# andrewhou1/BlindShadowRemoval

Hardware: AMD Instinct MI355X
Metric: images/sec at 256x256 batch inference (GSC generator forward) (higher is better)
Workload: dtype f32; 1 GPU; BASELINE configs[1]: batch=32 synthetic 256x256x3 per GPU, full GSC generator fp32 (seeded random-init weights in the ckpt-94 variable layout); global_batch=32, height=256, width=256, parallelism=dp1, forwards_in_flight=1, collective=none

## Files before the change

blindshadowremoval_amd/_lib.py:

```python
from __future__ import annotations

import ctypes
import os
from typing import Optional

from . import build as _build
from .build import LIB_PATH

ABI_VERSION = 8
NUM_CLASSES = 7
CLASS_NAMES = ("conv3x3", "convT3x3", "conv1x1", "attention", "conv7", "glue", "convT3x3_ni2")

_lib: Optional[ctypes.CDLL] = None

EXPORTS = ("bsr_create", "bsr_forward", "bsr_forward_tsm", "bsr_workspace_bytes", "bsr_reserve", "bsr_probe", "bsr_set_timing",
           "bsr_get_timing", "bsr_timing_launches", "bsr_timing_entry", "bsr_handle_workspace_bytes", "bsr_debug_attention", "bsr_debug_attention_dtype", "bsr_debug_attention_qw", "bsr_debug_split_qkv", "bsr_clock_trace", "bsr_debug_attention_split", "bsr_destroy", "bsr_last_error", "bsr_abi_version", "bsr_check_range", "bsr_prep_rows", "bsr_prep_groups", "bsr_png_unfilter", "bsr_forward_packed", "bsr_source_sha", "bsr_peek_range", "bsr_png_file_bytes", "bsr_png_scratch_bytes", "bsr_png_encode", "bsr_png_encode_figs", "bsr_ucb_post_scratch_bytes", "bsr_ucb_post",
           "bsr_forward_rgb", "bsr_debug_attention_rgb", "bsr_ucb_post_rgb_scratch_bytes", "bsr_ucb_post_rgb",
           "bsr_sfw_score_scratch_bytes", "bsr_sfw_score", "bsr_ucb_post_tsm_scratch_bytes", "bsr_ucb_post_tsm", "bsr_debug_wino_conv", "bsr_debug_wino_filter", "bsr_debug_keys_compose",
           "bsr_png_unfilter_tall", "bsr_crop_faces")


def load() -> ctypes.CDLL:
    global _lib
    if _lib is not None:
        return _lib
    if not os.path.isfile(LIB_PATH):
        raise RuntimeError("libbsr_hip.so is not built (%s missing): run `python -c 'import __graft_entry__ as g; g.build()'` "
                           "— the HIP path has no fallback" % LIB_PATH)
    try:
        import torch
    except ImportError:
        pass
    lib = ctypes.CDLL(LIB_PATH)
    try:
        lib.bsr_source_sha.restype = ctypes.c_char_p
        built = (lib.bsr_source_sha() or b"").decode()
    except AttributeError:
        built = "<none: built before the hash was embedded>"
    want = _build.source_sha16()
    if built != want:
        raise RuntimeError("libbsr_hip.so is STALE: it was compiled from kernel sources %s, the tree holds %s — rebuild "
                           "(`python -c 'import __graft_entry__ as g; g.build()'`); there is no fallback" % (built, want))
    c_f, c_i, c_v, c_sz = ctypes.POINTER(ctypes.c_float), ctypes.c_int, ctypes.c_void_p, ctypes.c_size_t
    lib.bsr_abi_version.restype = c_i
    lib.bsr_last_error.restype = ctypes.c_char_p
    lib.bsr_create.argtypes = [ctypes.POINTER(c_v), c_i, c_v, c_sz, c_i]
    lib.bsr_create.restype = c_i
    lib.bsr_forward.argtypes = [c_v, c_v, c_v, c_i, c_i, c_i, c_v, c_v, c_v, c_v, c_v]
    lib.bsr_forward.restype = c_i
    lib.bsr_forward_packed.argtypes = [c_v, c_v, c_v, c_i, c_i, c_i, c_v, c_v, c_v, c_v]
    lib.bsr_forward_packed.restype = c_i
    lib.bsr_forward_tsm.argtypes = [c_v, c_v, c_v, c_v, c_i, c_i, c_i, c_i, c_i, c_v, c_v, c_v, c_v, c_v]
    lib.bsr_forward_tsm.restype = c_i
    lib.bsr_forward_rgb.argtypes = [c_v, c_v, c_v, c_i, c_i, c_i, c_v, c_v]
    lib.bsr_forward_rgb.restype = c_i
    lib.bsr_debug_attention_rgb.argtypes = [c_v, c_v, c_i, c_i, c_v]
    lib.bsr_debug_attention_rgb.restype = c_i
    lib.bsr_workspace_bytes.argtypes = [c_i, c_i, c_i]
    lib.bsr_workspace_bytes.restype = c_sz
    lib.bsr_reserve.argtypes = [c_v, c_i, c_i, c_i]
    lib.bsr_reserve.restype = c_i
    lib.bsr_probe.argtypes = [c_v, ctypes.c_char_p, c_v, c_sz, ctypes.POINTER(c_i * 4), c_v]
    lib.bsr_probe.restype = c_i
    lib.bsr_set_timing.argtypes = [c_v, c_i]
    lib.bsr_set_timing.restype = c_i
    lib.bsr_get_timing.argtypes = [c_v, ctypes.POINTER(ctypes.c_float * NUM_CLASSES), ctypes.POINTER(c_i * NUM_CLASSES)]
    lib.bsr_get_timing.restype = c_i
    lib.bsr_timing_launches.argtypes = [c_v]
    lib.bsr_timing_launches.restype = c_i
    lib.bsr_timing_entry.argtypes = [c_v, c_i, ctypes.c_char_p, c_sz, ctypes.POINTER(ctypes.c_float), ctypes.POINTER(c_i)]
    lib.bsr_timing_entry.restype = c_i
    lib.bsr_handle_workspace_bytes.argtypes = [c_v, c_i, c_i, c_i]
    lib.bsr_handle_workspace_bytes.restype = c_sz
    lib.bsr_debug_attention.argtypes = [c_v, c_v, c_i, c_i, c_v]
    lib.bsr_debug_attention.restype = c_i
    lib.bsr_debug_attention_dtype.argtypes = [c_v, c_v, c_i, c_i, c_i, c_v]
    lib.bsr_debug_attention_dtype.restype = c_i
    lib.bsr_debug_attention_qw.argtypes = [c_v, c_v, c_i, c_i, c_i, c_v]
    lib.bsr_clock_trace.argtypes = [c_i, c_v, c_i, c_i, c_v, c_v, c_v]
    lib.bsr_clock_trace.restype = c_i
    lib.bsr_debug_split_qkv.argtypes = [c_v, c_v, c_i, c_i, c_v]
    lib.bsr_debug_split_qkv.restype = c_i
    lib.bsr_debug_attention_split.argtypes = [c_v, c_v, c_i, c_i, c_i, c_v]
    lib.bsr_debug_attention_split.restype = c_i
    lib.bsr_debug_attention_qw.restype = c_i
    lib.bsr_prep_rows.argtypes = [c_i, c_v, c_sz, c_sz, c_sz, c_i, c_i, c_v, c_v, c_v]
    lib.bsr_prep_rows.restype = c_i
    try:
        lib.bsr_prep_groups.argtypes = [c_i, c_v, c_sz, c_sz, c_sz, c_i, c_i, c_i, c_v, c_v, c_v]
    except AttributeError:
        raise RuntimeError("libbsr_hip.so has no bsr_prep_groups: rebuild (`python -c 'import __graft_entry__ as g; g.build()'`); "
                           "there is no fallback") from None
    lib.bsr_prep_groups.restype = c_i
    lib.bsr_png_unfilter.argtypes = [c_i, c_v, c_sz, c_sz, c_i, c_v]
    lib.bsr_png_unfilter.restype = c_i
    try:
        lib.bsr_png_unfilter_tall.argtypes = [c_i, c_v, c_sz, c_sz, c_i, c_v]
        lib.bsr_crop_faces.argtypes = [c_i, c_v, c_sz, c_sz, c_i, c_i, c_v]
    except AttributeError:
        raise RuntimeError("libbsr_hip.so has no bsr_png_unfilter_tall / bsr_crop_faces: rebuild (`python -c 'import __graft_entry__ as g; "
                           "g.build()'`); there is no fallback") from None
    lib.bsr_png_unfilter_tall.restype = c_i
    lib.bsr_crop_faces.restype = c_i
    lib.bsr_check_range.argtypes = [c_v, c_v]
    lib.bsr_check_range.restype = c_i
    lib.bsr_png_file_bytes.argtypes = [c_i, c_i]
    lib.bsr_png_file_bytes.restype = c_sz
    lib.bsr_png_scratch_bytes.argtypes = [c_i]
    lib.bsr_png_scratch_bytes.restype = c_sz
    lib.bsr_png_encode.argtypes = [c_i, c_v, c_i, c_i, c_i, c_v, c_sz, c_v, c_v]
    lib.bsr_png_encode.restype = c_i
    lib.bsr_png_encode_figs.argtypes = [c_i, c_i, c_v, c_v, c_v, c_v, c_v, c_v, c_i, c_i, c_i, c_v, c_sz, c_v, c_v]
    lib.bsr_png_encode_figs.restype = c_i
    lib.bsr_ucb_post_scratch_bytes.argtypes = [c_i, c_i]
    lib.bsr_ucb_post_scratch_bytes.restype = c_sz
    lib.bsr_ucb_post.argtypes = [c_i, c_v, c_v, c_v, c_i, c_i, c_v, c_v, c_v, c_v, c_v, c_v]
    lib.bsr_ucb_post.restype = c_i
    lib.bsr_ucb_post_rgb_scratch_bytes.argtypes = [c_i, c_i]
    lib.bsr_ucb_post_rgb_scratch_bytes.restype = c_sz
    lib.bsr_ucb_post_rgb.argtypes = [c_i, c_v, c_v, c_v, c_i, c_i, c_v, c_v, c_v, c_v, c_v, c_v]
    lib.bsr_ucb_post_rgb.restype = c_i
    lib.bsr_sfw_score_scratch_bytes.argtypes = [c_i, c_i]
    lib.bsr_sfw_score_scratch_bytes.restype = c_sz
    lib.bsr_sfw_score.argtypes = [c_i, c_v, c_i, c_i, c_v, c_v, c_v, c_v, c_v, c_v, c_v]
    lib.bsr_sfw_score.restype = c_i
    lib.bsr_ucb_post_tsm_scratch_bytes.argtypes = [c_i, c_i]
    lib.bsr_ucb_post_tsm_scratch_bytes.restype = c_sz
    lib.bsr_ucb_post_tsm.argtypes = [c_i, c_v, c_v, c_v, c_i, c_i, c_v, c_v, c_v, c_v, c_v, c_v, c_v]
    lib.bsr_ucb_post_tsm.restype = c_i
    lib.bsr_debug_wino_conv.argtypes = [c_v, c_v, c_v, c_v, c_i, c_i, c_i, c_i, c_v]
    lib.bsr_debug_wino_conv.restype = c_i
    lib.bsr_debug_wino_filter.argtypes = [c_v, c_v]
    lib.bsr_debug_wino_filter.restype = c_i
    try:
        lib.bsr_debug_keys_compose.argtypes = [c_v, c_v, c_v, c_v]
    except AttributeError:
        raise RuntimeError("libbsr_hip.so has no bsr_debug_keys_compose: rebuild (`python -c 'import __graft_entry__ as g; g.build()'`); "
                           "there is no fallback") from None
    lib.bsr_debug_keys_compose.restype = c_i
    lib.bsr_peek_range.argtypes = [c_v]
    lib.bsr_peek_range.restype = c_i
    lib.bsr_destroy.argtypes = [c_v]
    lib.bsr_destroy.restype = None
    if lib.bsr_abi_version() != ABI_VERSION:
        raise RuntimeError("libbsr_hip.so ABI %d != binding ABI %d: rebuild" % (lib.bsr_abi_version(), ABI_VERSION))
    _lib = lib
    return lib


def source_sha() -> str:
    return (load().bsr_source_sha() or b"").decode()


class RangeError(RuntimeError):
    """BSR_ERR_RANGE: an activation did not fit fp16 in a forward of a 16-bit-mode handle (include/bsr_hip.h, bsr_check_range)."""


ERR_RANGE = 5


def check(rc: int, what: str) -> None:
    if rc != 0:
        msg = load().bsr_last_error()
        raise (RangeError if rc == ERR_RANGE else RuntimeError)("%s failed (code %d): %s" % (what, rc, msg.decode() if msg else "?"))
```

blindshadowremoval_amd/csrc/attention.h:

```cpp
#pragma once
#include <hip/hip_runtime.h>
#include <type_traits>
#include "igemm_conv.h"
#include "gemm_tail.h"

#ifndef BSR_ATT_PRIO
#define BSR_ATT_PRIO 0
#endif

namespace bsr {

constexpr int kAttD = 128;
constexpr int kAttKT = 32;
constexpr int kAttLdK = kAttD + 4;
constexpr float kRescaleThreshold = 8.f;
constexpr int kAttStageFloats = kAttKT * kAttLdK + kAttKT * kAttD;
constexpr int kAttSmemBytes = 4 * kAttStageFloats * 4;
static_assert(kAttSmemBytes <= 160 * 1024, "LDS budget");
static_assert(66 * 64 * 4 <= 4 * kAttStageFloats, "merge scratch fits the staging buffers");

typedef GemmTailArgs AttWArgs;
typedef GemmTailCfg<5, 4> AttWCfg;
constexpr int kAttWSmemBytes = AttWCfg::SMEM_FLOATS * 4;
static_assert(kAttWSmemBytes <= 160 * 1024 && kAttWSmemBytes >= kAttSmemBytes, "LDS budget of the fused tail");
static_assert(4 * 66 * 64 <= kTailAFloats && kTailLdA == kAttLdK, "the merge scratch sits under the attention tile, clear of the weight ring");

template <int QW, bool FUSEW = false>
__global__ __launch_bounds__(QW * 128, QW == 4 ? 2 : 1) void nonlocal_attention_kernel(const float* __restrict__ qkv, float* __restrict__ out, int tokens, AttWArgs wa) {
  static_assert(!FUSEW || QW == 4, "the fused w tail is the 8-wave shape's");
  extern __shared__ __attribute__((aligned(16))) float smem[];
  constexpr int NT = QW * 128;
  constexpr int SV = 2048 / NT;
  const int tid = threadIdx.x, lane = tid & 63;
  const int wave = __builtin_amdgcn_readfirstlane(tid >> 6);
  const int grp = wave / QW, wq = wave % QW;
  const int h = lane >> 5, r = lane & 31;
  const int qblocks = tokens / (QW * 32);
  int img, qb;
  {
    const int nblk = gridDim.x, b = blockIdx.x;
    const int per_round = 8 * qblocks;
    if (nblk % per_round == 0) {
      const int round = b / per_round, within = b % per_round;
      img = round * 8 + (within % 8);
      qb = within / 8;
    } else {
      img = b / qblocks;
      qb = b % qblocks;
    }
  }
  const float* base = qkv + (size_t)img * tokens * (3 * kAttD);
  const int q = qb * (QW * 32) + wq * 32 + r;
#if BSR_ATT_PRIO
  if (grp == (BSR_ATT_PRIO - 1)) __builtin_amdgcn_s_setprio(2); else __builtin_amdgcn_s_setprio(0);
#endif

  f32x4 qf[kAttD / 8];
#pragma unroll
  for (int g = 0; g < kAttD / 8; ++g)
    qf[g] = *reinterpret_cast<const f32x4*>(base + (size_t)q * (3 * kAttD) + g * 8 + 4 * h) * 1.4426950408889634f;

  f32x16 o[4];
#pragma unroll
  for (int dt = 0; dt < 4; ++dt)
#pragma unroll
    for (int i = 0; i < 16; ++i) o[dt][i] = 0.f;
  float m_run = -INFINITY, l_run = 0.f;

  constexpr int V4_PER_TILE = kAttKT * kAttD / 4;
  constexpr int NV = V4_PER_TILE / NT;
  f32x4 kreg[SV], vreg[SV];
  typedef unsigned u32x4_t __attribute__((ext_vector_type(4)));
  const __amdgpu_buffer_rsrc_t kv_rsrc = make_rsrc(base);
  unsigned kv_voff[NV];
#pragma unroll
  for (int i = 0; i < NV; ++i) {
    const int idx = (tid + i * NT) & (V4_PER_TILE - 1);
    kv_voff[i] = (unsigned)(((idx / (kAttD / 4)) * (3 * kAttD) + (idx % (kAttD / 4)) * 4) * 4);
  }
  auto fetch = [&](int pr) {
#pragma unroll
    for (int i = 0; i < SV; ++i) {
      const unsigned soff = (unsigned)((2 * pr + (i / NV)) * kAttKT * (3 * kAttD) * 4);
      kreg[i] = __builtin_bit_cast(f32x4, (u32x4_t)__builtin_amdgcn_raw_buffer_load_b128(kv_rsrc, kv_voff[i % NV] + (unsigned)(kAttD * 4), soff, 0));
      vreg[i] = __builtin_bit_cast(f32x4, (u32x4_t)__builtin_amdgcn_raw_buffer_load_b128(kv_rsrc, kv_voff[i % NV] + (unsigned)(2 * kAttD * 4), soff, 0));
    }
  };
  auto publish = [&](int pbuf) {
#pragma unroll
    for (int i = 0; i < SV; ++i) {
      const int idx = (tid + i * NT) & (V4_PER_TILE - 1), sel = (tid + i * NT) >> 10;
      const int key = idx / (kAttD / 4), c4 = idx % (kAttD / 4);
      float* sk = smem + (2 * pbuf + sel) * kAttStageFloats;
      float* sv = sk + kAttKT * kAttLdK;
      *reinterpret_cast<f32x4*>(sk + key * kAttLdK + c4 * 4) = kreg[i];
      *reinterpret_cast<f32x4*>(sv + key * kAttD + c4 * 4) = vreg[i];
    }
  };

  const int npair = tokens / (2 * kAttKT);
  fetch(0);
  publish(0);
  __syncthreads();

  auto pair_step = [&](int pr, auto pbuf_const) {
    constexpr int pbuf = decltype(pbuf_const)::value;
    if (pr + 1 < npair) fetch(pr + 1);
    const float* sk = smem + (2 * pbuf + grp) * kAttStageFloats;
    const float* sv = sk + kAttKT * kAttLdK;

    f32x16 s;
#pragma unroll
    for (int i = 0; i < 16; ++i) s[i] = 0.f;
#pragma unroll
    for (int g = 0; g < kAttD / 8; ++g) {
      const f32x4 kf = *reinterpret_cast<const f32x4*>(sk + r * kAttLdK + g * 8 + 4 * h);
#pragma unroll
      for (int j = 0; j < 4; ++j) s = __builtin_amdgcn_mfma_f32_32x32x2f32(kf[j], qf[g][j], s, 0, 0, 0);
    }

    float mx = s[0];
#pragma unroll
    for (int i = 1; i < 16; ++i) mx = fmaxf(mx, s[i]);
    mx = fmaxf(mx, __shfl_xor(mx, 32));
    if (__any(mx > m_run + kRescaleThreshold)) {
      const float m_new = fmaxf(m_run, mx);
      const float scale = __builtin_amdgcn_exp2f(m_run - m_new);
      l_run *= scale;
      m_run = m_new;
#pragma unroll
      for (int dt = 0; dt < 4; ++dt)
#pragma unroll
        for (int i = 0; i < 16; ++i) o[dt][i] *= scale;
    }
    f32x2 ps2 = {0.f, 0.f};
    const f32x2 m2 = {m_run, m_run};
#pragma unroll
    for (int i = 0; i < 16; i += 2) {
      const f32x2 d = f32x2{s[i], s[i + 1]} - m2;
      s[i] = __builtin_amdgcn_exp2f(d[0]);
      s[i + 1] = __builtin_amdgcn_exp2f(d[1]);
      ps2 += f32x2{s[i], s[i + 1]};
    }
    l_run += ps2[0] + ps2[1];

#pragma unroll
    for (int i = 0; i < 16; ++i) {
      const int key = (i & 3) + 8 * (i >> 2) + 4 * h;
      const f32x4 vf = *reinterpret_cast<const f32x4*>(sv + key * kAttD + 4 * r);
#pragma unroll
      for (int dt = 0; dt < 4; ++dt) o[dt] = __builtin_amdgcn_mfma_f32_32x32x2f32(vf[dt], s[i], o[dt], 0, 0, 0);
    }

    if (pr + 1 < npair) {
      publish(pbuf ^ 1);
      __syncthreads();
    }
  };
  for (int pr = 0; pr < npair; pr += 2) {
    pair_step(pr, std::integral_constant<int, 0>{});
    pair_step(pr + 1, std::integral_constant<int, 1>{});
  }

  __syncthreads();
  [[maybe_unused]] float* s_ring = smem + kTailAFloats;
  [[maybe_unused]] float* s_bias = s_ring + 3 * kTailSlot;
  [[maybe_unused]] GemmTailState<5, 4> tail;
  if constexpr (FUSEW) gemm_tail_prefetch(tail, wa, s_bias, tid);
  float* sx = smem + (size_t)wq * 66 * 64 + lane;
  if (grp == 1) {
    sx[0] = m_run;
    sx[64] = l_run;
#pragma unroll
    for (int dt = 0; dt < 4; ++dt)
#pragma unroll
      for (int i = 0; i < 16; ++i) sx[(2 + dt * 16 + i) * 64] = o[dt][i];
  }
  __syncthreads();
  if constexpr (!FUSEW) {
    if (grp == 1) return;
  }
  float inv = 0.f;
  if (grp == 0) {
    const float m1 = sx[0], l1 = sx[64];
    const float m = fmaxf(m_run, m1);
    const float s0 = __builtin_amdgcn_exp2f(m_run - m), s1 = __builtin_amdgcn_exp2f(m1 - m);
    l_run = l_run * s0 + l1 * s1;
#pragma unroll
    for (int dt = 0; dt < 4; ++dt)
#pragma unroll
      for (int i = 0; i < 16; ++i) o[dt][i] = o[dt][i] * s0 + sx[(2 + dt * 16 + i) * 64] * s1;
    const float l_tot = l_run + __shfl_xor(l_run, 32);
    inv = 1.f / l_tot;
  }

  if constexpr (!FUSEW) {
    float* orow = out + ((size_t)img * tokens + q) * kAttD;
#pragma unroll
    for (int i = 0; i < 16; ++i) {
      const int row = (i & 3) + 8 * (i >> 2) + 4 * h;
      f32x4 v = {o[0][i] * inv, o[1][i] * inv, o[2][i] * inv, o[3][i] * inv};
      *reinterpret_cast<f32x4*>(orow + 4 * row) = v;
    }
  } else {
    __syncthreads();
    float* s_att = smem;
    if (grp == 0) {
      float* arow = s_att + (wq * 32 + r) * kTailLdA;
#pragma unroll
      for (int i = 0; i < 16; ++i) {
        const int row = (i & 3) + 8 * (i >> 2) + 4 * h;
        f32x4 v = {o[0][i] * inv, o[1][i] * inv, o[2][i] * inv, o[3][i] * inv};
        *reinterpret_cast<f32x4*>(arow + 4 * row) = v;
      }
    }
    const size_t tile_pix = (size_t)img * tokens + (size_t)qb * 128 + (size_t)__builtin_amdgcn_readfirstlane(wq) * 32;
    gemm_tail_run(tail, wa, s_att, s_ring, s_bias, grp, wq, tile_pix, lane);
  }
}

template <int QW>
inline hipError_t launch_nonlocal_attention_qw(const float* qkv, float* out, int batch, int tokens, hipStream_t stream) {
  auto kern = nonlocal_attention_kernel<QW, false>;
  static PerDeviceOnce once;
  const int dev = PerDeviceOnce::current();
  if (dev < 0 || !once.done[dev]) {
    hipError_t e = hipFuncSetAttribute(reinterpret_cast<const void*>(kern), hipFuncAttributeMaxDynamicSharedMemorySize, kAttSmemBytes);
    if (e != hipSuccess) return e;
    if (dev >= 0) once.done[dev] = true;
  }
  hipLaunchKernelGGL(kern, dim3(batch * (tokens / (QW * 32))), dim3(QW * 128), kAttSmemBytes, stream, qkv, out, tokens, AttWArgs{});
  return hipGetLastError();
}

inline int attention_auto_qw(int batch, int tokens) {
  const long long cus = device_cu_count();
  const long long blocks128 = (long long)batch * (tokens / 128);
  long long best = -1;
  int qw = 4;
  for (int cand : {4, 2, 1}) {
    const long long rounds = (blocks128 * (4 / cand) + cus - 1) / cus;
    const long long cost = rounds * (cand == 4 ? 17 : 10);
    if (best < 0 || cost < best) { best = cost; qw = cand; }
  }
  return qw;
}

inline hipError_t launch_nonlocal_attention_w(const float* qkv, int batch, int tokens, const AttWArgs& wa, hipStream_t stream) {
  if (tokens % (4 * kAttKT) != 0 || wa.n_pad * 32 < AttWCfg::BIAS_FLOATS * 32 || wa.n_pad < 12 * 32 || wa.n_store > 288 || wa.res_c > 288 || wa.out2 != nullptr) return hipErrorInvalidValue;
  auto kern = nonlocal_attention_kernel<4, true>;
  static PerDeviceOnce once;
  const int dev = PerDeviceOnce::current();
  if (dev < 0 || !once.done[dev]) {
    hipError_t e = hipFuncSetAttribute(reinterpret_cast<const void*>(kern), hipFuncAttributeMaxDynamicSharedMemorySize, kAttWSmemBytes);
    if (e != hipSuccess) return e;
    if (dev >= 0) once.done[dev] = true;
  }
  hipLaunchKernelGGL(kern, dim3(batch * (tokens / 128)), dim3(512), kAttWSmemBytes, stream, qkv, static_cast<float*>(nullptr), tokens, wa);
  return hipGetLastError();
}

inline hipError_t launch_nonlocal_attention(const float* qkv, float* out, int batch, int tokens, hipStream_t stream, int qw = 0) {
  if (tokens % (4 * kAttKT) != 0) return hipErrorInvalidValue;
  if (qw == 0) qw = attention_auto_qw(batch, tokens);
  if (qw == 4) return launch_nonlocal_attention_qw<4>(qkv, out, batch, tokens, stream);
  if (qw == 2) return launch_nonlocal_attention_qw<2>(qkv, out, batch, tokens, stream);
  if (qw == 1) return launch_nonlocal_attention_qw<1>(qkv, out, batch, tokens, stream);
  return hipErrorInvalidValue;
}

}
```

blindshadowremoval_amd/csrc/bsr_api.hip:

```cpp
#include "../../include/bsr_hip.h"

#include <hip/hip_runtime.h>
#include <stdint.h>
#include <stdio.h>
#include <stdlib.h>
#include <string.h>

#include <initializer_list>
#include <string>
#include <type_traits>
#include <unordered_map>
#include <vector>

#include "attention.h"
#include "attention256.h"
#include "attention_h16.h"
#include "conv3_f16.h"
#include "conv_n16.h"
#include "gemm_nloop.h"
#include "glue_kernels.h"
#include "igemm_conv.h"
#include "igemm_h16.h"
#include "png_kernels.h"
#include "prep_kernels.h"
#include "prep_group_kernels.h"
#include "rgb_head.h"
#include "stem7.h"
#include "ucb_kernels.h"
#include "ucb_rgb_kernels.h"
#include "ucb_tsm_kernels.h"
#include "sfw_kernels.h"
#include "wino_conv2.h"
#include "wild_crop_kernels.h"

namespace {

thread_local std::string g_last_error;

int fail(int code, const std::string& msg) {
  g_last_error = msg;
  return code;
}

#define HIP_TRY(expr)                                                                              \
  do {                                                                                             \
    hipError_t e__ = (expr);                                                                       \
    if (e__ != hipSuccess)                                                                         \
      return fail(BSR_ERR_HIP, std::string(#expr) + ": " + hipGetErrorString(e__));                \
  } while (0)

struct DeviceGuard {
  int prev = -1;
  hipError_t err = hipSuccess;
  explicit DeviceGuard(int device) {
    if (hipGetDevice(&prev) != hipSuccess) prev = -1;
    if (prev != device) err = hipSetDevice(device);
  }
  ~DeviceGuard() {
    if (prev >= 0) (void)hipSetDevice(prev);
  }
};

bool post_size_ok(int B, int S) { return B > 0 && (S == 32 || S == 64 || S == 128 || S == 256); }

template <class Launch>
int run_post(const char* name, std::initializer_list<const void*> required, int B, int S, const void* scratch, int device, Launch launch) {
  for (const void* p : required)
    if (p == nullptr) return fail(BSR_ERR_ARG, std::string(name) + ": null argument");
  if (!post_size_ok(B, S)) return fail(BSR_ERR_ARG, std::string(name) + ": B must be positive and S one of 32, 64, 128, 256 (reference: 256)");
  if (reinterpret_cast<uintptr_t>(scratch) % 256 != 0) return fail(BSR_ERR_ARG, std::string(name) + ": scratch must be 256-byte aligned");
  DeviceGuard guard(device);
  HIP_TRY(guard.err);
  return launch();
}

constexpr uint32_t kBlobMagic = 0x57525342u;
constexpr uint32_t kBlobVersion = 1;
struct BlobHeader {
  uint32_t magic, version, n_entries, reserved;
};
struct BlobEntry {
  char name[40];
  uint64_t offset;
  uint64_t nfloats;
  int32_t dims[4];
};

struct LayerW {
  const float* w = nullptr;
  const float* b = nullptr;
  int nchunk = 0, taps = 0, n_pad = 0, ldp = 0;
};

enum KClass { K_CONV3 = 0, K_CONVT = 1, K_CONV1 = 2, K_ATT = 3, K_CONV7 = 4, K_GLUE = 5, K_CONVT_NI2 = 6 };

struct Variant {
  bool tsm, rgb;
  int c_a, cs_a, uv_a;
  int c_r, cs_r;
  int c_h, cs_h, uv_h;
  int d = 128, nblk = 6;
  int cs_c3 = 128, cs_c2 = 160;
  int cs_y3x = 288;
  int cs_y = 64, cs_qh = 16;
};
constexpr Variant kGSC{false, false, 99, 120, 96, 257, 264, 261, 264, 258};
constexpr Variant kGSC16{false, false, 99, 128, 96, 257, 288, 261, 288, 258};
constexpr Variant kTSM{true, false, 291, 312, 288, 291, 312, 877, 888, 874};
constexpr Variant kTSM16{true, false, 291, 320, 288, 291, 320, 877, 896, 874};
constexpr Variant kRGB{false, true, 99, 128, 96, 513, 544, 0, 0, 0, 256, 3, 192, 256, 544, 128, 32};
constexpr int CS_Y3X = kGSC.cs_y3x;
constexpr int CS_CF = 64;
constexpr int RGB_CS_R = kRGB.cs_r, RGB_CS_A = kRGB.cs_a, RGB_D = kRGB.d, RGB_CS_C3 = kRGB.cs_c3, RGB_CS_C2 = kRGB.cs_c2, RGB_CS_QH = kRGB.cs_qh;

struct Region {
  size_t off, floats;
};
struct Plan {
  size_t x1, c3, c2, xa, t1, t2, y3[6], qkv, att[6], r[6], xh, ybuf, qh, f1, f2, cf, probe, reg32, share, yh, con, total;
  Region zero[8];
  int nzero;
};

Plan make_plan(size_t B, size_t H, size_t W, const Variant& v) {
  Plan p{};
  size_t off = 0;
  auto take = [&](size_t floats, bool keep_zero = false) {
    size_t o = off;
    off += (floats + 63) & ~size_t(63);
    if (keep_zero && floats != 0) p.zero[p.nzero++] = {o, floats};
    return o;
  };
  const size_t px = B * H * W, cells = px / 64;
  const size_t px2 = v.rgb ? 0 : px;
  const size_t px1 = px - px2;
  p.x1 = take(px * 32);
  p.c3 = take(px / 4 * v.cs_c3);
  p.c2 = take(px / 16 * v.cs_c2);
  p.xa = take(cells * v.cs_a, true);
  p.t1 = take(cells * v.d);
  p.t2 = take(cells * v.d);
  for (int i = 0; i < v.nblk; ++i) p.y3[i] = take(cells * v.cs_y3x);
  p.qkv = take(cells * 3 * v.d);
  for (int i = 0; i < v.nblk; ++i) p.att[i] = take(cells * v.d);
  for (int i = 0; i < v.nblk; ++i) p.r[i] = take(cells * (i < 3 ? v.cs_r : v.cs_h), !v.rgb);
  p.xh = take(cells * v.cs_h, true);
  p.ybuf = take(px * v.cs_y);
  p.qh = take(px * v.cs_qh);
  p.f1 = take(px2 / 16 * 128);
  p.f2 = take(px2 / 4 * 96);
  p.cf = take(px2 * CS_CF);
  p.probe = take(px2 / 64 * 2);
  p.reg32 = take(v.tsm ? cells * 4 : 0);
  p.share = take(v.tsm ? cells * 2 * v.c_r : 0);
  p.yh = take(px1 * 3);
  p.con = take(px1 * 3);
  p.total = off;
  return p;
}

}

struct bsr_handle {
  int device = 0;
  float* d_blob = nullptr;
  float* d_wino = nullptr;
  float* d_keys = nullptr;
  std::unordered_map<std::string, LayerW> layers;
  Variant var = kGSC;
  int dtype = BSR_DTYPE_F32;
  float head_bias[2] = {0.f, 0.f};
  const float* tail_w = nullptr;
  const float* clr_gs_w = nullptr;
  float* ws = nullptr;
  size_t ws_floats = 0;
  Plan plan{};
  const float* rgb_tail_w = nullptr;
  const float* rgb_head_b = nullptr;
  int B = 0, H = 0, W = 0;
  bool ran = false;
  bool att_in_lds = false;
  unsigned* range_flag = nullptr;
  bool fuse_heads = true;
  bool conv1_gemm = true;
  bool att_pv1 = false;
  bool conv3_f16 = true;
  bool fuse_attw = true;
  bool wino_conv2 = true;
  bool keys_conv2 = true;
  bool timing = false;
  std::vector<hipEvent_t> ev;
  std::vector<int> ev_class;
  std::vector<std::string> ev_name;
  size_t ev_used = 0;
};

namespace {

const char* const kRangeMsg =
    "an activation exceeded the fp16 range (|x| >= 65520) in a forward of this 16-bit-mode handle: its outputs are not trustworthy "
    "(inf / NaN where the fp32 path stays finite).  Re-run those inputs on a BSR_DTYPE_F32 handle; bsr_check_range() clears the condition";

constexpr size_t kWinoFloats = 8 * 16 * 128 * 16;
void wino_filter_transform(const float* direct, float* out) {
  static const double G[4][3] = {{1.0, 0.0, 0.0}, {0.5, 0.5, 0.5}, {0.5, -0.5, 0.5}, {0.0, 0.0, 1.0}};
  for (int k = 0; k < 128; ++k)
    for (int n = 0; n < 128; ++n) {
      double t[4][3];
      for (int x = 0; x < 4; ++x)
        for (int b = 0; b < 3; ++b) {
          double acc = 0.0;
          for (int a = 0; a < 3; ++a) acc += G[x][a] * (double)direct[((size_t)((k / 32) * 9 + a * 3 + b) * 128 + n) * 36 + k % 32];
          t[x][b] = acc;
        }
      for (int x = 0; x < 4; ++x)
        for (int y = 0; y < 4; ++y) {
          double acc = 0.0;
          for (int b = 0; b < 3; ++b) acc += t[x][b] * G[y][b];
          out[((size_t)((k / 16) * 16 + 4 * x + y) * 128 + n) * 16 + k % 16] = (float)acc;
        }
    }
}

constexpr int kKeysN = 288 + 256, kKeysNPad = kKeysN + 64, kC3qNPad = 768;
constexpr size_t kKeysFloats = (size_t)4 * kKeysNPad * 36 + kKeysNPad;
void keys_compose(const float* c3q_w, const float* c3q_b, float* out_w, float* out_b) {
  auto src = [&](int k, int n) -> const float& { return c3q_w[((size_t)(k / 32) * kC3qNPad + n) * 36 + k % 32]; };
  memset(out_w, 0, (size_t)4 * kKeysNPad * 36 * sizeof(float));
  memset(out_b, 0, kKeysNPad * sizeof(float));
  for (int ch = 0; ch < 4; ++ch) {
    memcpy(out_w + (size_t)ch * kKeysNPad * 36, c3q_w + (size_t)ch * kC3qNPad * 36, (size_t)288 * 36 * sizeof(float));
    memcpy(out_w + ((size_t)ch * kKeysNPad + 416) * 36, c3q_w + ((size_t)ch * kC3qNPad + 544) * 36, (size_t)128 * 36 * sizeof(float));
  }
  memcpy(out_b, c3q_b, 288 * sizeof(float));
  memcpy(out_b + 416, c3q_b + 544, 128 * sizeof(float));
  for (int m = 0; m < 128; ++m) {
    for (int k = 0; k < 128; ++k) {
      double acc = 0.0;
      for (int c = 0; c < 128; ++c) acc += (double)src(k, 288 + c) * (double)src(m, 416 + c);
      out_w[((size_t)(k / 32) * kKeysNPad + 288 + m) * 36 + k % 32] = (float)acc;
    }
    double acc = 0.0;
    for (int c = 0; c < 128; ++c) acc += (double)c3q_b[288 + c] * (double)src(m, 416 + c);
    out_b[288 + m] = (float)acc;
  }
}

int find_layer(bsr_handle* h, const char* name, int nchunk, int taps, int ldp, int n_min, LayerW* out) {
  auto it = h->layers.find(name);
  if (it == h->layers.end()) return fail(BSR_ERR_BLOB, std::string("blob has no layer '") + name + "'");
  const LayerW& l = it->second;
  if (l.w == nullptr || l.b == nullptr || l.nchunk != nchunk || l.taps != taps || l.ldp != ldp || l.n_pad < n_min) {
    char buf[256];
    snprintf(buf, sizeof buf, "layer '%s': blob has {chunks %d, taps %d, n_pad %d, ldp %d}, kernel needs {%d, %d, >=%d, %d}", name,
             l.nchunk, l.taps, l.n_pad, l.ldp, nchunk, taps, n_min, ldp);
    return fail(BSR_ERR_BLOB, buf);
  }
  *out = l;
  return BSR_OK;
}

template <int V>
using int_c = std::integral_constant<int, V>;
template <class F>
void with_dtype(int dtype, F f) {
  if (dtype == BSR_DTYPE_F32) f(int_c<0>{}, std::false_type{});
  else if (dtype == BSR_DTYPE_F16) f(int_c<2>{}, std::true_type{});
  else f(int_c<2>{}, std::false_type{});
}
template <class F>
void with_io(int io, F f) {
  if (io == 3) f(int_c<3>{});
  else if (io == 2) f(int_c<2>{});
  else if (io == 1) f(int_c<1>{});
  else f(int_c<0>{});
}

bsr::WinoArgs wino_args(const float* in, float* out, const float* w, const float* bias, int H, int W, int out_cs = 128) {
  bsr::WinoArgs a{};
  a.in = in; a.out = out; a.w = w; a.bias = bias; a.H = H; a.W = W; a.in_cs = 128; a.out_cs = out_cs; a.act = 1;
  return a;
}

struct Launcher {
  bsr_handle* h;
  hipStream_t s;
  int rc = BSR_OK;

  void begin(int cls, const char* name) {
    if (!h->timing) return;
    if (h->ev_used + 2 > h->ev.size()) {
      for (int i = 0; i < 2; ++i) {
        hipEvent_t e;
        if (hipEventCreate(&e) != hipSuccess) return;
        h->ev.push_back(e);
      }
      h->ev_class.push_back(cls);
      h->ev_name.emplace_back();
    }
    h->ev_class[h->ev_used / 2] = cls;
    h->ev_name[h->ev_used / 2] = name;
    hipEventRecord(h->ev[h->ev_used], s);
  }
  void end() {
    if (!h->timing || h->ev_used + 2 > h->ev.size()) return;
    hipEventRecord(h->ev[h->ev_used + 1], s);
    h->ev_used += 2;
  }
  void check(hipError_t e, const char* what) {
    if (e != hipSuccess && rc == BSR_OK) rc = fail(BSR_ERR_HIP, std::string(what) + ": " + hipGetErrorString(e));
  }

  template <int KH, int KW, int S, bool TR, int NI, int CC, int INB>
  void conv(int cls, const char* name, const float* in, int in_cs, int in_coff, int k_pad, int H, int W, float* out, int out_cs,
            int out_coff, int n_store, int act, int io = 0) {
    if (rc != BSR_OK) return;
    using C = bsr::ConvCfg<KH, KW, S, TR, 4, 32, 4, 1, 1, NI, CC, INB>;
    constexpr bool k33 = (KH == 3 && KW == 3);
    constexpr bool k11 = (KH == 1 && KW == 1);
    constexpr int CCH = CC == 24 ? 32 : CC;
    const bool h16 = h->dtype != BSR_DTYPE_F32;
    const int nsplit = (k33 && h->dtype == BSR_DTYPE_F16) ? 1 : 2;
    LayerW l;
    const int nb = (n_store + C::BN - 1) / C::BN;
    if (h16) {
      if (k_pad % CCH != 0) { rc = fail(BSR_ERR_ARG, std::string("layer '") + name + "': K is not a multiple of the 16-bit kernels' chunk"); return; }
      const int ldpw = nsplit == 2 ? bsr::H16Cfg<KH, KW, S, TR, 4, 32, 4, 1, 1, NI, CCH, INB, 2>::LDPW : (CCH + 8) / 2;
      rc = find_layer(h, name, k_pad / CCH, KH * KW, ldpw, nb * C::BN, &l);
    } else {
      rc = find_layer(h, name, k_pad / CC, KH * KW, CC + 4, nb * C::BN, &l);
    }
    if (rc != BSR_OK) return;
    bsr::ConvArgs a{};
    a.in = in; a.in_cs = in_cs; a.in_coff = in_coff; a.H = H; a.W = W;
    a.out = out; a.out_cs = out_cs; a.out_coff = out_coff;
    a.Ho = TR ? 2 * H : (H + S - 1) / S;
    a.Wo = TR ? 2 * W : (W + S - 1) / S;
    a.w = l.w; a.bias = l.b; a.nchunk = l.nchunk; a.n_pad = l.n_pad; a.n_store = n_store;
    auto pad_before = [](int in, int k, int s) {
      int o = (in + s - 1) / s, tot = (o - 1) * s + k - in;
      return tot > 0 ? tot / 2 : 0;
    };
    a.pad_t = pad_before(H, KH, S);
    a.pad_l = pad_before(W, KW, S);
    a.act = act;
    a.range_flag = h->range_flag;
    const int mh = TR ? H : a.Ho, mw = TR ? W : a.Wo;
    if (mh % 4 != 0 || mw % 32 != 0) {
      rc = fail(BSR_ERR_ARG, std::string("layer '") + name + "': feature map is not a multiple of the 4x32 tile");
      return;
    }
    if constexpr (k33 && S == 1) {
      if (h->dtype == BSR_DTYPE_F16 && h->conv3_f16) {
        char nm3[48];
        snprintf(nm3, sizeof nm3, "%s.w3", name);
        LayerW l3;
        const int nblk = (n_store + 63) / 64;
        rc = find_layer(h, nm3, nblk * (k_pad / 32), 9, 16, 64, &l3);
        if (rc != BSR_OK) return;
        a.w = l3.w; a.bias = l3.b; a.nchunk = k_pad / 32; a.n_pad = nblk * 64;
        begin(cls, name);
        with_io(io, [&](auto io_c) { check(bsr::launch_conv3_f16<TR, io_c.value>(a, h->B, s), name); });
        end();
        return;
      }
    }
    begin(cls, name);
    static_assert(k33 || k11, "igemm layers are 3x3 or 1x1");
    constexpr bool kTrunk = !TR && S == 1 && NI == 2 && (CC == 32 || (k11 && CC == 24));
    bool half_tile = false;
    if constexpr (kTrunk) half_tile = !h16 && mh % 2 == 0 && (long long)(mh / 4) * (mw / 32) * h->B * nb < bsr::device_cu_count();
    if (half_tile) {
      if constexpr (kTrunk) check(bsr::launch_igemm_conv<KH, KW, S, TR, 2, 32, 2, 2, 1, 1, CC, INB>(a, h->B, s), name);
    } else if (!h16)
      check(bsr::launch_igemm_conv<KH, KW, S, TR, 4, 32, 4, 1, 1, NI, CC, INB>(a, h->B, s), name);
    else if (nsplit == 2)
      check(bsr::launch_igemm_h16<KH, KW, S, TR, 4, 32, 4, 1, 1, NI, CCH, INB, 2>(a, h->B, s), name);
    else if constexpr (k33)
      with_io(io, [&](auto io_c) { check(bsr::launch_igemm_h16<KH, KW, S, TR, 4, 32, 4, 1, 1, NI, CCH, INB, 1, io_c.value>(a, h->B, s), name); });
    end();
  }
  bsr::ConvArgs gemm_args(const LayerW& l, const float* in, int in_cs, float* out, int out_cs, int n_store, int act) const {
    bsr::ConvArgs a{};
    a.in = in; a.in_cs = in_cs; a.out = out; a.out_cs = out_cs;
    a.w = l.w; a.bias = l.b; a.nchunk = l.nchunk; a.n_pad = l.n_pad; a.n_store = n_store; a.act = act;
    a.range_flag = h->range_flag;
    return a;
  }
  template <int NI, int NCH, int MINW = 2>
  void gemm(int cls, const char* name, const float* in, int in_cs, size_t pixels, float* out, int out_cs, int n_store, int act,
            const float* res1 = nullptr, int res1_cs = 0, int res1_c = 0,
            float* out2 = nullptr, int out2_cs = 0, int n_split = 0, int n_store1 = 0, const LayerW* image = nullptr, int out2_gap_at = 0,
            int out2_gap = 0) {
    if (rc != BSR_OK) return;
    using C = bsr::GemmNLoopCfg<NI, NCH>;
    LayerW l;
    const int tiles = (n_store + 31) / 32;
    int kNSplit = 2;
    {
      const long long mblocks = (long long)(pixels / C::BM);
      const int want = (int)((2LL * bsr::device_cu_count() + mblocks - 1) / (mblocks > 0 ? mblocks : 1));
      const int most = (tiles + NI - 1) / NI;
      kNSplit = want < 2 ? 2 : (want > most ? most : want);
#ifdef BSR_NL_NSPLIT
      kNSplit = BSR_NL_NSPLIT > most ? most : BSR_NL_NSPLIT;
#endif
    }
    if (image == nullptr) rc = find_layer(h, name, NCH, 1, 36, (tiles + NI - 1) * 32, &l);
    else if (image->nchunk == NCH && image->ldp == 36 && image->n_pad >= (tiles + NI - 1) * 32) l = *image;
    else rc = fail(BSR_ERR_ARG, std::string("layer '") + name + "': the handle's image does not fit the kernel");
    if (rc != BSR_OK) return;
    if (pixels % C::BM != 0) { rc = fail(BSR_ERR_ARG, std::string("layer '") + name + "': pixel count is not a multiple of 128"); return; }
    bsr::ConvArgs a = gemm_args(l, in, in_cs, out, out_cs, n_store, act);
    a.res1 = res1; a.res1_cs = res1_cs; a.res1_c = res1_c;
    a.out2 = out2; a.out2_cs = out2_cs; a.n_split = n_split; a.n_store1 = n_store1; a.out2_gap_at = out2_gap_at; a.out2_gap = out2_gap;
    a.out2_split = (h->dtype != BSR_DTYPE_F32 && out2 != nullptr) ? 1 : 0;
    begin(cls, name);
    if (h->dtype == BSR_DTYPE_F32)
      check(bsr::launch_gemm_nloop<NI, NCH, 0, MINW>(a, pixels, kNSplit, s), name);
    else if constexpr (MINW == 2)
      check(bsr::launch_gemm_nloop<NI, NCH, 2>(a, pixels, kNSplit, s), name);
    else
      rc = fail(BSR_ERR_ARG, std::string("layer '") + name + "': the RGB bottleneck GEMMs are fp32 only");
    end();
  }
  template <int NCH>
  void gemm_all_n(const char* name, const float* in, size_t pixels, float* out) {
    if (rc != BSR_OK) return;
    LayerW l;
    rc = find_layer(h, name, NCH, 1, 36, 128, &l);
    if (rc != BSR_OK) return;
    begin(K_CONV1, name);
    check(bsr::launch_gemm_nloop<4, NCH, 2, 1>(gemm_args(l, in, NCH * 32, out, 128, 128, 1), pixels, 1, s), name);
    end();
  }

  void stem(const float* in, int H, int W, float* out) {
    if (rc != BSR_OK) return;
    LayerW l;
    rc = find_layer(h, "conv1", 1, 7, h->dtype != BSR_DTYPE_F32 ? 36 : 28, 32, &l);
    if (rc != BSR_OK) return;
    bsr::StemArgs a{in, out, l.w, l.b, H, W, 0, 0, 0, h->range_flag};
    begin(K_CONV7, "conv1");
    with_dtype(h->dtype, [&](auto prec, auto half) { check(bsr::launch_stem7<4, prec.value, half.value>(a, h->B, s), "conv1"); });
    end();
  }

  void wino(const char* name, int i, const float* in, int H, int W, float* out, int out_cs = 128) {
    if (rc != BSR_OK) return;
    LayerW l;
    rc = find_layer(h, name, 4, 9, 36, 128, &l);
    if (rc != BSR_OK) return;
    if (H % 4 != 0 || W % 32 != 0) { rc = fail(BSR_ERR_ARG, std::string("layer '") + name + "': feature map is not a multiple of the 4x32 tile"); return; }
    begin(K_CONV3, name);
    check(bsr::launch_wino_conv2(wino_args(in, out, h->d_wino + (size_t)i * kWinoFloats, l.b, H, W, out_cs), h->B, s), name);
    end();
  }

  void conv71(const char* name, const float* in, int in_cs, int k_pad, int H, int W, float* out, int out_cs) {
    if (rc != BSR_OK) return;
    LayerW l;
    rc = find_layer(h, name, k_pad / 32, 7, 36, 32, &l);
    if (rc != BSR_OK) return;
    if (H % 4 != 0 || W % 32 != 0) { rc = fail(BSR_ERR_ARG, std::string("layer '") + name + "': image is not a multiple of the 4x32 tile"); return; }
    bsr::ConvArgs a{};
    a.in = in; a.in_cs = in_cs; a.in_coff = 0; a.H = H; a.W = W;
    a.out = out; a.out_cs = out_cs; a.out_coff = 0; a.Ho = H; a.Wo = W;
    a.w = l.w; a.bias = l.b; a.nchunk = l.nchunk; a.n_pad = l.n_pad; a.n_store = 32;
    a.pad_t = 3; a.pad_l = 0; a.act = 0;
    begin(K_CONV7, name);
    check(bsr::launch_igemm_conv<7, 1, 1, false, 4, 32, 4, 1, 1, 1, 32, 1>(a, h->B, s), name);
    end();
  }

  void heads(const float* y, int H, int W, float* qh, const float* inputs, float* gs, float* mask22, size_t npix) {
    if (rc != BSR_OK) return;
    LayerW l;
    rc = find_layer(h, "heads", 2, 7, 36, 16, &l);
    if (rc != BSR_OK) return;
    if (l.n_pad != 16) { rc = fail(BSR_ERR_BLOB, "layer 'heads' must be packed with n_pad 16"); return; }
    if (H % 8 != 0 || W % 32 != 0) { rc = fail(BSR_ERR_ARG, "layer 'heads': image is not a multiple of its tile"); return; }
    bsr::ConvN16Args a{};
    a.in = y; a.in_cs = 64; a.H = H; a.W = W; a.w = l.w; a.bias = l.b; a.out = qh; a.out_cs = 16; a.act = 0;
    a.pad_t = 3; a.pad_l = 0;
    a.inputs = inputs; a.gs_out = gs; a.mask22 = mask22; a.b_mask = h->head_bias[0]; a.b_con = h->head_bias[1];
    a.range_flag = h->range_flag;
    int resident = 0;
    check(bsr::launch_conv_n16<7, 1, false, false, 2, 0, false, true>(a, h->B, s, &resident), "heads");
    const bool fuse = rc == BSR_OK && h->fuse_heads && bsr::conv_n16_fuse_pays(h->B, H, 8, resident);
    begin(K_CONV7, "heads");
    with_dtype(h->dtype, [&](auto prec, auto half) {
      if (fuse) check(bsr::launch_conv_n16<7, 1, false, false, 2, prec.value, half.value, true>(a, h->B, s), "heads");
      else check(bsr::launch_conv_n16<7, 1, false, false, 2, prec.value, half.value>(a, h->B, s), "heads");
    });
    end();
    if (fuse) return;
    begin(K_GLUE, "heads_post");
    hipLaunchKernelGGL(bsr::heads_post_kernel, dim3((unsigned)((npix + 255) / 256)), dim3(256), 0, s, qh, inputs, h->head_bias[0], h->head_bias[1], gs,
                       mask22, W, npix);
    check(hipGetLastError(), "heads_post");
    end();
  }

  template <int KH, int KW, bool GS, bool TAIL, int RW>
  void conv16(int cls, const char* name, const float* in, int in_cs, int H, int W, float* out, int out_cs, int act, const float* gs,
              const float* inputs, float* con_rgb, float* dif, float* packed = nullptr) {
    if (rc != BSR_OK) return;
    LayerW l;
    rc = find_layer(h, name, 2, KH * KW, 36, 16, &l);
    if (rc != BSR_OK) return;
    if (l.n_pad != 16) { rc = fail(BSR_ERR_BLOB, std::string("layer '") + name + "' must be packed with n_pad 16"); return; }
    bsr::ConvN16Args a{};
    a.in = in; a.in_cs = in_cs; a.H = H; a.W = W; a.w = l.w; a.bias = l.b; a.out = out; a.out_cs = out_cs; a.act = act;
    a.pad_t = (KH - 1) / 2; a.pad_l = (KW - 1) / 2;
    a.gs = gs; a.w_gs = h->clr_gs_w; a.tail_w = h->tail_w; a.inputs = inputs; a.con_rgb = con_rgb; a.dif = dif; a.packed = packed;
    a.range_flag = h->range_flag;
    if (H % (4 * RW) != 0 || W % 32 != 0) { rc = fail(BSR_ERR_ARG, std::string("layer '") + name + "': image is not a multiple of its tile"); return; }
    begin(cls, name);
    with_dtype(h->dtype, [&](auto prec, auto half) { check(bsr::launch_conv_n16<KH, KW, GS, TAIL, RW, prec.value, half.value>(a, h->B, s), name); });
    end();
  }
};

int grow_workspace(bsr_handle* h, size_t floats, bool device_wide, hipStream_t s) {
  if (floats <= h->ws_floats) return BSR_OK;
  if (device_wide) HIP_TRY(hipDeviceSynchronize());
  else HIP_TRY(hipStreamSynchronize(s));
  if (h->ws) HIP_TRY(hipFree(h->ws));
  h->ws = nullptr;
  h->ws_floats = 0;
  HIP_TRY(hipMalloc(reinterpret_cast<void**>(&h->ws), floats * sizeof(float)));
  h->ws_floats = floats;
  h->B = 0;
  h->ran = false;
  if (device_wide) HIP_TRY(hipMemset(h->ws, 0, floats * sizeof(float)));
  else HIP_TRY(hipMemsetAsync(h->ws, 0, floats * sizeof(float), s));
  return BSR_OK;
}

int ensure_workspace(bsr_handle* h, int B, int H, int W, hipStream_t s) {
  const Plan p = make_plan(B, H, W, h->var);
  const bool fresh = p.total > h->ws_floats;
  const int rc = grow_workspace(h, p.total, false, s);
  if (rc != BSR_OK) return rc;
  if (!fresh && (B != h->B || H != h->H || W != h->W)) {
    for (int i = 0; i < p.nzero; ++i) HIP_TRY(hipMemsetAsync(h->ws + p.zero[i].off, 0, p.zero[i].floats * sizeof(float), s));
    h->ran = false;
  }
  h->plan = p;
  h->B = B; h->H = H; h->W = W;
  return BSR_OK;
}

template <typename T>
int read_records(const unsigned char* blob, size_t off, int n, hipStream_t s, std::vector<T>* out) {
  out->resize((size_t)n);
  HIP_TRY(hipMemcpyAsync(out->data(), blob + off, (size_t)n * sizeof(T), hipMemcpyDeviceToHost, s));
  HIP_TRY(hipStreamSynchronize(s));
  return BSR_OK;
}

}

extern "C" {

int bsr_abi_version(void) { return 8; }

#ifndef BSR_SRC_SHA
#define BSR_SRC_SHA "unhashed"
#endif
static const char kSrcShaTag[] = "BSR_SRC_SHA=" BSR_SRC_SHA;
const char* bsr_source_sha(void) { return kSrcShaTag + 12; }

const char* bsr_last_error(void) { return g_last_error.c_str(); }

size_t bsr_workspace_bytes(int B, int H, int W) {
  if (B <= 0 || H <= 0 || W <= 0) return 0;
  return make_plan(B, H, W, kGSC).total * sizeof(float);
}

int bsr_create(bsr_handle** out, int device, const void* packed_weights, size_t nbytes, int dtype) {
  if (out == nullptr || packed_weights == nullptr) return fail(BSR_ERR_ARG, "bsr_create: null argument");
  *out = nullptr;
  if (dtype != BSR_DTYPE_F32 && dtype != BSR_DTYPE_F16 && dtype != BSR_DTYPE_F32X3)
    return fail(BSR_ERR_ARG, "bsr_create: dtype must be BSR_DTYPE_F32, BSR_DTYPE_F16 or BSR_DTYPE_F32X3");
  if (nbytes < sizeof(BlobHeader)) return fail(BSR_ERR_BLOB, "bsr_create: blob shorter than its header");
  const uint8_t* blob = static_cast<const uint8_t*>(packed_weights);
  BlobHeader hd;
  memcpy(&hd, blob, sizeof hd);
  if (hd.magic != kBlobMagic || hd.version != kBlobVersion) return fail(BSR_ERR_BLOB, "bsr_create: bad blob magic/version");
  if ((int)hd.reserved != dtype) return fail(BSR_ERR_BLOB, "bsr_create: the blob was packed for another dtype (pack_generator(weights, dtype) must match bsr_create's dtype)");
  const size_t table_end = sizeof(BlobHeader) + (size_t)hd.n_entries * sizeof(BlobEntry);
  if (table_end > nbytes) return fail(BSR_ERR_BLOB, "bsr_create: blob entry table exceeds blob size");
  DeviceGuard guard(device);
  HIP_TRY(guard.err);
  bsr_handle* h = new bsr_handle();
  h->device = device;
  h->dtype = dtype;
  h->att_pv1 = dtype == BSR_DTYPE_F16;
  const struct { const char* env; bool* on; } switches[] = {{"BSR_FUSE_HEADS", &h->fuse_heads}, {"BSR_FUSE_ATTW", &h->fuse_attw}, {"BSR_CONV3_F16", &h->conv3_f16},
                                                            {"BSR_CONV1_GEMM", &h->conv1_gemm}, {"BSR_WINO_CONV2", &h->wino_conv2},
                                                            {"BSR_KEYS_CONV2", &h->keys_conv2}};
  for (const auto& sw : switches)
    if (const char* e_ = getenv(sw.env)) *sw.on = atoi(e_) != 0;
  hipError_t e = hipMalloc(reinterpret_cast<void**>(&h->d_blob), nbytes);
  if (e == hipSuccess) e = hipMemcpy(h->d_blob, blob, nbytes, hipMemcpyHostToDevice);
  if (e != hipSuccess) {
    if (h->d_blob) hipFree(h->d_blob);
    delete h;
    return fail(BSR_ERR_HIP, std::string("bsr_create: weight upload: ") + hipGetErrorString(e));
  }
  for (uint32_t i = 0; i < hd.n_entries; ++i) {
    BlobEntry en;
    memcpy(&en, blob + sizeof(BlobHeader) + (size_t)i * sizeof(BlobEntry), sizeof en);
    en.name[sizeof(en.name) - 1] = 0;
    if (en.offset % 16 != 0 || en.offset + en.nfloats * 4 > nbytes) {
      bsr_destroy(h);
      return fail(BSR_ERR_BLOB, std::string("bsr_create: entry '") + en.name + "' is out of bounds or misaligned");
    }
    std::string nm(en.name);
    const float* dptr = reinterpret_cast<const float*>(reinterpret_cast<const uint8_t*>(h->d_blob) + en.offset);
    if (nm == "heads.bias") {
      if (en.nfloats != 2) { bsr_destroy(h); return fail(BSR_ERR_BLOB, "bsr_create: heads.bias must hold 2 floats"); }
      memcpy(h->head_bias, blob + en.offset, 8);
    } else if (nm == "clr_conv1.gs") {
      if (en.nfloats != 256) { bsr_destroy(h); return fail(BSR_ERR_BLOB, "bsr_create: clr_conv1.gs must hold 16x16 floats"); }
      h->clr_gs_w = dptr;
    } else if (nm == "rgb.tail") {
      if (en.nfloats != 7 * 7 * 3 * 3 + 3) { bsr_destroy(h); return fail(BSR_ERR_BLOB, "bsr_create: rgb.tail must hold 7x7x3x3 + 3 floats"); }
      h->rgb_tail_w = dptr;
    } else if (nm == "rgb.head_bias") {
      if (en.nfloats != 3) { bsr_destroy(h); return fail(BSR_ERR_BLOB, "bsr_create: rgb.head_bias must hold 3 floats"); }
      h->rgb_head_b = dptr;
    } else if (nm == "tail.w") {
      if (en.nfloats != 16 * 16 + 16 + 48 + 3) { bsr_destroy(h); return fail(BSR_ERR_BLOB, "bsr_create: tail.w has the wrong size"); }
      h->tail_w = dptr;
    } else if (nm.size() > 2 && nm.compare(nm.size() - 2, 2, ".w") == 0) {
      LayerW& l = h->layers[nm.substr(0, nm.size() - 2)];
      l.w = dptr;
      l.nchunk = en.dims[0]; l.taps = en.dims[1]; l.n_pad = en.dims[2]; l.ldp = en.dims[3];
      if ((uint64_t)l.nchunk * l.taps * l.n_pad * l.ldp != en.nfloats) {
        bsr_destroy(h);
        return fail(BSR_ERR_BLOB, std::string("bsr_create: entry '") + en.name + "' dims do not match its size");
      }
    } else if (nm.size() > 2 && nm.compare(nm.size() - 2, 2, ".b") == 0) {
      h->layers[nm.substr(0, nm.size() - 2)].b = dptr;
    }
  }
  if (h->layers.count("rgb_head") != 0) {
    if (dtype != BSR_DTYPE_F32) {
      bsr_destroy(h);
      return fail(BSR_ERR_ARG, "bsr_create: these are RGB-baseline weights (model_RGB.py), which run in BSR_DTYPE_F32 only: BSR_DTYPE_F32X3 and BSR_DTYPE_F16 are not provided for them");
    }
    if (h->rgb_tail_w == nullptr || h->rgb_head_b == nullptr) { bsr_destroy(h); return fail(BSR_ERR_BLOB, "bsr_create: RGB blob lacks 'rgb.tail' / 'rgb.head_bias'"); }
    h->var = kRGB;
    *out = h;
    return BSR_OK;
  }
  if (h->tail_w == nullptr || h->clr_gs_w == nullptr) { bsr_destroy(h); return fail(BSR_ERR_BLOB, "bsr_create: blob lacks 'tail.w' / 'clr_conv1.gs'"); }
  if (dtype != BSR_DTYPE_F32) {
    e = hipHostMalloc(reinterpret_cast<void**>(&h->range_flag), 64, hipHostMallocMapped);
    if (e != hipSuccess) { h->range_flag = nullptr; bsr_destroy(h); return fail(BSR_ERR_HIP, std::string("bsr_create: range flag: ") + hipGetErrorString(e)); }
    *h->range_flag = 0u;
  }
  {
    auto it = h->layers.find("res0.conv1");
    if (it == h->layers.end()) { bsr_destroy(h); return fail(BSR_ERR_BLOB, "bsr_create: blob has no 'res0.conv1'"); }
    const int nch = it->second.nchunk;
    if (dtype == BSR_DTYPE_F32) h->var = nch == 13 ? kTSM : kGSC;
    else h->var = nch == 10 ? kTSM16 : kGSC16;
  }
  if (dtype == BSR_DTYPE_F32) {
    std::vector<float> u(6 * kWinoFloats);
    for (int i = 0; i < 6; ++i) {
      char nm[32];
      snprintf(nm, sizeof nm, "res%d.conv2", i);
      LayerW l;
      if (find_layer(h, nm, 4, 9, 36, 128, &l) != BSR_OK || l.n_pad != 128) { bsr_destroy(h); return fail(BSR_ERR_BLOB, std::string("bsr_create: layer '") + nm + "' is not a [4][9][128][36] image"); }
      wino_filter_transform(reinterpret_cast<const float*>(blob + (reinterpret_cast<const uint8_t*>(l.w) - reinterpret_cast<const uint8_t*>(h->d_blob))), u.data() + i * kWinoFloats);
    }
    e = hipMalloc(reinterpret_cast<void**>(&h->d_wino), u.size() * sizeof(float));
    if (e == hipSuccess) e = hipMemcpy(h->d_wino, u.data(), u.size() * sizeof(float), hipMemcpyHostToDevice);
    if (e != hipSuccess) { bsr_destroy(h); return fail(BSR_ERR_HIP, std::string("bsr_create: Winograd weights: ") + hipGetErrorString(e)); }
    std::vector<float> q(6 * kKeysFloats);
    auto host = [&](const float* dev) { return reinterpret_cast<const float*>(blob + (reinterpret_cast<const uint8_t*>(dev) - reinterpret_cast<const uint8_t*>(h->d_blob))); };
    for (int i = 0; i < 6; ++i) {
      char nm[32];
      snprintf(nm, sizeof nm, "res%d.c3q", i);
      LayerW l;
      if (find_layer(h, nm, 4, 1, 36, kC3qNPad, &l) != BSR_OK || l.n_pad != kC3qNPad) { bsr_destroy(h); return fail(BSR_ERR_BLOB, std::string("bsr_create: layer '") + nm + "' is not a [4][1][768][36] image"); }
      keys_compose(host(l.w), host(l.b), q.data() + i * kKeysFloats, q.data() + i * kKeysFloats + (size_t)4 * kKeysNPad * 36);
    }
    e = hipMalloc(reinterpret_cast<void**>(&h->d_keys), q.size() * sizeof(float));
    if (e == hipSuccess) e = hipMemcpy(h->d_keys, q.data(), q.size() * sizeof(float), hipMemcpyHostToDevice);
    if (e != hipSuccess) { bsr_destroy(h); return fail(BSR_ERR_HIP, std::string("bsr_create: composed c3q weights: ") + hipGetErrorString(e)); }
  }
  *out = h;
  return BSR_OK;
}

void bsr_destroy(bsr_handle* h) {
  if (h == nullptr) return;
  DeviceGuard guard(h->device);
  for (hipEvent_t e : h->ev) hipEventDestroy(e);
  if (h->ws) hipFree(h->ws);
  if (h->d_blob) hipFree(h->d_blob);
  if (h->d_wino) hipFree(h->d_wino);
  if (h->d_keys) hipFree(h->d_keys);
  if (h->range_flag) hipHostFree(h->range_flag);
  delete h;
}

int bsr_reserve(bsr_handle* h, int B, int H, int W) {
  if (h == nullptr || B <= 0 || H <= 0 || W <= 0) return fail(BSR_ERR_ARG, "bsr_reserve: bad argument");
  DeviceGuard guard(h->device);
  HIP_TRY(guard.err);
  return grow_workspace(h, make_plan(B, H, W, h->var).total, true, nullptr);
}

int bsr_check_range(bsr_handle* h, void* stream) {
  if (h == nullptr) return fail(BSR_ERR_ARG, "bsr_check_range: null handle");
  if (h->range_flag == nullptr) return BSR_OK;
  DeviceGuard guard(h->device);
  HIP_TRY(guard.err);
  HIP_TRY(hipStreamSynchronize(static_cast<hipStream_t>(stream)));
  if (__atomic_exchange_n(h->range_flag, 0u, __ATOMIC_SEQ_CST) == 0u) return BSR_OK;
  return fail(BSR_ERR_RANGE, kRangeMsg);
}

int bsr_peek_range(bsr_handle* h) {
  if (h == nullptr) return fail(BSR_ERR_ARG, "bsr_peek_range: null handle");
  if (h->range_flag == nullptr) return BSR_OK;
  if (__atomic_load_n(h->range_flag, __ATOMIC_SEQ_CST) == 0u) return BSR_OK;
  return fail(BSR_ERR_RANGE, kRangeMsg);
}

int bsr_set_timing(bsr_handle* h, int enable) {
  if (h == nullptr) return fail(BSR_ERR_ARG, "bsr_set_timing: null handle");
  h->timing = enable != 0;
  h->ev_used = 0;
  return BSR_OK;
}

int bsr_get_timing(bsr_handle* h, float ms[BSR_NUM_CLASSES], int launches[BSR_NUM_CLASSES]) {
  if (h == nullptr || ms == nullptr || launches == nullptr) return fail(BSR_ERR_ARG, "bsr_get_timing: null argument");
  for (int i = 0; i < BSR_NUM_CLASSES; ++i) { ms[i] = 0.f; launches[i] = 0; }
  for (size_t i = 0; i + 1 < h->ev_used; i += 2) {
    HIP_TRY(hipEventSynchronize(h->ev[i + 1]));
    float t = 0.f;
    HIP_TRY(hipEventElapsedTime(&t, h->ev[i], h->ev[i + 1]));
    const int c = h->ev_class[i / 2];
    ms[c] += t;
    launches[c] += 1;
  }
  return BSR_OK;
}

int bsr_timing_launches(bsr_handle* h) { return h == nullptr ? 0 : (int)(h->ev_used / 2); }

int bsr_timing_entry(bsr_handle* h, int i, char* name, size_t name_cap, float* ms, int* cls) {
  if (h == nullptr || name == nullptr || ms == nullptr || cls == nullptr || name_cap == 0) return fail(BSR_ERR_ARG, "bsr_timing_entry: null argument");
  if (i < 0 || (size_t)(2 * i + 1) >= h->ev_used) return fail(BSR_ERR_ARG, "bsr_timing_entry: index out of range");
  HIP_TRY(hipEventSynchronize(h->ev[2 * i + 1]));
  HIP_TRY(hipEventElapsedTime(ms, h->ev[2 * i], h->ev[2 * i + 1]));
  *cls = h->ev_class[i];
  snprintf(name, name_cap, "%s", h->ev_name[i].c_str());
  return BSR_OK;
}

size_t bsr_handle_workspace_bytes(const bsr_handle* h, int B, int H, int W) {
  if (h == nullptr || B <= 0 || H <= 0 || W <= 0) return 0;
  return make_plan(B, H, W, h->var).total * sizeof(float);
}

static int check_image_size(int H, int W, const char* hw_text, const char* token_text) {
  if (H <= 0 || W <= 0 || H % 32 != 0 || W % 256 != 0) return fail(BSR_ERR_ARG, hw_text);
  if (((H / 8) * (W / 8)) % 128 != 0) return fail(BSR_ERR_ARG, token_text);
  return BSR_OK;
}
#define BSR_CHECK_IMAGE_SIZE(entry, H, W)                                                                                          \
  check_image_size(H, W, entry ": H must be a multiple of 32 and W a multiple of 256 (reference: 256x256)",                         \
                   entry ": (H/8)*(W/8) must be a multiple of 128")

static int forward_impl(bsr_handle* h, const float* inputs, const float* uv, const float* reg, int frame, int share, int B, int H, int W,
                        float* gs, float* con_rgb, float* mask22, float* dif, void* stream, float* packed = nullptr) {
  if (h == nullptr || inputs == nullptr || uv == nullptr || gs == nullptr || mask22 == nullptr || (packed == nullptr && (con_rgb == nullptr || dif == nullptr)))
    return fail(BSR_ERR_ARG, "bsr_forward: null argument");
  if (B <= 0) return fail(BSR_ERR_ARG, "bsr_forward: B must be positive");
  const Variant& V = h->var;
  if (V.rgb)
    return fail(BSR_ERR_ARG, reg != nullptr ? "bsr_forward_tsm: this handle holds RGB-baseline weights: call bsr_forward_rgb"
                                            : "bsr_forward: this handle holds RGB-baseline weights: call bsr_forward_rgb");
  if (V.tsm != (reg != nullptr))
    return fail(BSR_ERR_ARG, V.tsm ? "bsr_forward: this handle holds TSM weights: call bsr_forward_tsm" : "bsr_forward_tsm: this handle holds GSC weights: call bsr_forward");
  if (V.tsm && (frame <= 0 || B % frame != 0 || H != W))
    return fail(BSR_ERR_ARG, "bsr_forward_tsm: B must be a multiple of frame and the image square (warp.py assumes a square map)");
  int rc = BSR_CHECK_IMAGE_SIZE("bsr_forward", H, W);
  if (rc != BSR_OK) return rc;
  hipStream_t s = static_cast<hipStream_t>(stream);
  if (h->range_flag != nullptr && *reinterpret_cast<volatile unsigned*>(h->range_flag) != 0u)
    return fail(BSR_ERR_RANGE, kRangeMsg);
  DeviceGuard guard(h->device);
  HIP_TRY(guard.err);
  rc = ensure_workspace(h, B, H, W, s);
  if (rc != BSR_OK) return rc;
  h->ev_used = 0;
  const Plan& p = h->plan;
  float* ws = h->ws;
  const size_t npix = (size_t)B * H * W, ncell = npix / 64;
  const int H2 = H / 2, W2 = W / 2, H4 = H / 4, W4 = W / 4, H8 = H / 8, W8 = W / 8;
  Launcher L{h, s};
  auto glue_begin = [&](const char* what) { L.begin(K_GLUE, what); };
  auto glue_end = [&](const char* what) { L.check(hipGetLastError(), what); L.end(); };

  L.stem(inputs, H, W, ws + p.x1);
  const bool p16 = h->dtype == BSR_DTYPE_F16;
  const int io_both = p16 ? 3 : 0, io_in = p16 ? 1 : 0, io_out = p16 ? 2 : 0;
  L.conv<3, 3, 2, false, 2, 16, 1>(K_CONV3, "down1", ws + p.x1, 32, 0, 32, H, W, ws + p.c3, 128, 64, 64, 1, io_both);
  L.conv<3, 3, 2, false, 2, 16, 1>(K_CONV3, "down2", ws + p.c3, 128, 64, 64, H2, W2, ws + p.c2, 160, 96, 64, 1, io_both);
  L.conv<3, 3, 2, false, 3, 16, 1>(K_CONV3, "down3", ws + p.c2, 160, 96, 64, H4, W4, ws + p.xa, V.cs_a, 0, 96, 1, io_in);
  glue_begin("uv_resize8");
  hipLaunchKernelGGL(bsr::uv_resize8_kernel, dim3((unsigned)((ncell * 3 + 255) / 256)), dim3(256), 0, s, uv, H, W, ws + p.xa, V.cs_a, V.uv_a,
                     ws + p.xh, V.cs_h, V.uv_h, ncell);
  glue_end("uv_resize8");

  auto share_layer = [&](const float* x, int x_cs, int C, float* out, int out_cs, int out_coff) {
    glue_begin("share_layer");
    if (share) hipLaunchKernelGGL(bsr::share_reduce_kernel, dim3((unsigned)(ncell / frame)), dim3(128), 0, s, x, x_cs, C, ws + p.reg32, H8, frame, ws + p.share);
    hipLaunchKernelGGL(bsr::share_unwarp_kernel, dim3((unsigned)ncell), dim3(128), 0, s, ws + p.share, x, x_cs, C, ws + p.reg32, H8, frame, share, out, out_cs, out_coff);
    glue_end("share_layer");
  };
  if (V.tsm) {
    glue_begin("reg_resize8");
    hipLaunchKernelGGL(bsr::reg_resize8_kernel, dim3((unsigned)((ncell * 4 + 255) / 256)), dim3(256), 0, s, reg, H, W, ws + p.reg32, ncell);
    glue_end("reg_resize8");
    share_layer(ws + p.xa, V.cs_a, 96, ws + p.xa, V.cs_a, 96);
  }

  auto conv1_gemm = [&](const char* nm, const float* x, int x_cs) -> bool {
    if (V.tsm || !h->conv1_gemm || L.rc != BSR_OK) return false;
    if (h->dtype == BSR_DTYPE_F32) return false;
    if (ncell % 128 != 0 || (long long)(ncell / 128) * 2 < bsr::device_cu_count()) return false;
    if (x_cs != 128 && x_cs != 288) return false;
    if (x_cs == 128) L.gemm_all_n<4>(nm, x, ncell, ws + p.t1);
    else L.gemm_all_n<9>(nm, x, ncell, ws + p.t1);
    return true;
  };

  auto res_block = [&](int i, const float* x, int x_cs, int x_c) {
    float* r_out = ws + p.r[i];
    const int o_cs = i < 3 ? V.cs_r : V.cs_h;
    char nm[32];
    float* y3 = ws + p.y3[i];
    snprintf(nm, sizeof nm, "res%d.conv1", i);
    if (!conv1_gemm(nm, x, x_cs)) L.conv<1, 1, 1, false, 2, 24, 3>(K_CONV1, nm, x, x_cs, 0, x_cs, H8, W8, ws + p.t1, 128, 0, 128, 1);
    const bool keys = h->dtype == BSR_DTYPE_F32 && h->keys_conv2;
    float* t2_row = keys ? ws + p.qkv : ws + p.t2;
    const int t2_cs = keys ? 384 : 128, t2_coff = keys ? 128 : 0;
    float* t2 = t2_row + t2_coff;
    snprintf(nm, sizeof nm, "res%d.conv2", i);
    if (h->dtype == BSR_DTYPE_F32 && h->wino_conv2) L.wino(nm, i, ws + p.t1, H8, W8, t2, t2_cs);
    else L.conv<3, 3, 1, false, 2, 32, 1>(K_CONV3, nm, ws + p.t1, 128, 0, 128, H8, W8, t2_row, t2_cs, t2_coff, 128, 1);
    snprintf(nm, sizeof nm, "res%d.c3q", i);
    if (keys) {
      const float* img = h->d_keys + (size_t)i * kKeysFloats;
      const LayerW lk{img, img + (size_t)4 * kKeysNPad * 36, 4, 1, kKeysNPad, 36};
      L.gemm<3, 4>(K_CONV1, nm, t2, t2_cs, ncell, y3, CS_Y3X, kKeysN, 0, x, x_cs, x_cs < 288 ? x_cs : 288, ws + p.qkv, 384, 288, CS_Y3X, &lk, 128, 128);
    } else {
      L.gemm<3, 4>(K_CONV1, nm, t2, t2_cs, ncell, y3, CS_Y3X, 288 + 384, 0, x, x_cs, x_cs < 288 ? x_cs : 288, ws + p.qkv, 384, 288, CS_Y3X);
    }
    const bool h16 = h->dtype != BSR_DTYPE_F32;
    const bool fuse_w = h->fuse_attw && (h16 || bsr::attention_auto_qw(B, H8 * W8) == 4);
    h->att_in_lds = fuse_w;
    if (fuse_w && L.rc == BSR_OK) {
      LayerW l;
      snprintf(nm, sizeof nm, h16 ? "res%d.w4" : "res%d.w", i);
      L.rc = h16 ? find_layer(h, nm, 9, 1, 128, 32, &l) : find_layer(h, nm, 4, 1, 36, 12 * 32, &l);
      if (L.rc == BSR_OK) {
        bsr::AttWArgs wa{};
        wa.w = l.w; wa.bias = l.b; wa.n_pad = h16 ? 288 : l.n_pad;
        wa.res = y3; wa.res_cs = CS_Y3X; wa.res_c = CS_Y3X;
        wa.out = r_out; wa.out_cs = o_cs; wa.n_store = o_cs < 288 ? o_cs : 288; wa.n_store1 = wa.n_store; wa.act = 1; wa.stagger = 1;
        snprintf(nm, sizeof nm, "res%d.attw", i);
        L.begin(K_ATT, nm);
        if (!h16)
          L.check(bsr::launch_nonlocal_attention_w(ws + p.qkv, B, H8 * W8, wa, s), "attention+w");
        else
          L.check(bsr::launch_nonlocal_attention_h16_w(ws + p.qkv, B, H8 * W8, wa, s, h->att_pv1), "attention_h16+w");
        L.end();
      }
    } else {
      if (L.rc == BSR_OK) {
        snprintf(nm, sizeof nm, "res%d.attention", i);
        L.begin(K_ATT, nm);
        if (!h16)
          L.check(bsr::launch_nonlocal_attention(ws + p.qkv, ws + p.att[i], B, H8 * W8, s), "attention");
        else
          L.check(bsr::launch_nonlocal_attention_h16(ws + p.qkv, ws + p.att[i], B, H8 * W8, s, h->att_pv1), "attention_h16");
        L.end();
      }
      snprintf(nm, sizeof nm, "res%d.w", i);
      L.gemm<3, 4>(K_CONV1, nm, ws + p.att[i], 128, ncell, r_out, o_cs, o_cs < 288 ? o_cs : 288, 1, y3, CS_Y3X, CS_Y3X);
    }
    if (x_c > 288 && L.rc == BSR_OK) {
      glue_begin("lrelu_copy");
      hipLaunchKernelGGL(bsr::lrelu_copy_kernel, dim3((unsigned)((ncell * (x_c - 288) + 255) / 256)), dim3(256), 0, s, x, x_cs, r_out, o_cs, 288, x_c, ncell);
      glue_end("lrelu_copy");
    }
  };
  res_block(0, ws + p.xa, V.cs_a, V.c_a);
  res_block(1, ws + p.r[0], V.cs_r, V.c_r);
  res_block(2, ws + p.r[1], V.cs_r, V.c_r);

  L.conv<3, 3, 1, true, 1, 24, 1>(K_CONVT, "up1", ws + p.r[2], V.cs_r, 0, V.cs_r, H8, W8, ws + p.c2, 160, 0, 96, 1, io_out);
  L.conv<3, 3, 1, true, 2, 32, 1>(K_CONVT_NI2, "up2", ws + p.c2, 160, 0, 160, H4, W4, ws + p.c3, 128, 0, 64, 1, io_both);
  L.conv<3, 3, 1, true, 2, 32, 1>(K_CONVT_NI2, "up3", ws + p.c3, 128, 0, 128, H2, W2, ws + p.ybuf, 64, 0, 64, 1, io_both);
  L.heads(ws + p.ybuf, H, W, ws + p.qh, inputs, gs, mask22, npix);
  glue_begin("bmask_xhole");
  hipLaunchKernelGGL(bsr::bmask_xhole_kernel, dim3((unsigned)ncell), dim3(64), 0, s, gs, inputs, H, W, ws + p.r[2], V.cs_r, V.c_r, ws + p.xh,
                     V.cs_h, ws + p.probe);
  glue_end("bmask_xhole");
  if (V.tsm) share_layer(ws + p.xh, V.cs_h, V.c_r, ws + p.xh, V.cs_h, V.c_r + 1);

  res_block(3, ws + p.xh, V.cs_h, V.c_h);
  res_block(4, ws + p.r[3], V.cs_h, V.c_h);
  res_block(5, ws + p.r[4], V.cs_h, V.c_h);

  L.conv<3, 3, 1, true, 2, 24, 1>(K_CONVT, "clr_up1", ws + p.r[5], V.cs_h, 0, V.cs_h, H8, W8, ws + p.f1, 128, 0, 128, 1, io_out);
  L.conv<3, 3, 1, true, 1, 32, 1>(K_CONVT, "clr_up2", ws + p.f1, 128, 0, 128, H4, W4, ws + p.f2, 96, 0, 96, 1, io_both);
  L.conv<3, 3, 1, true, 2, 32, 1>(K_CONVT_NI2, "clr_up3", ws + p.f2, 96, 0, 96, H2, W2, ws + p.cf, CS_CF, 0, 64, 1, io_both);
  L.conv16<3, 3, true, true, 2>(K_CONV3, "clr_conv1", ws + p.cf, CS_CF, H, W, nullptr, 0, 1, gs, inputs, con_rgb, dif, packed);
  if (L.rc == BSR_OK) h->ran = true;
  return L.rc;
}

int bsr_forward_rgb(bsr_handle* h, const float* inputs, const float* uv, int B, int H, int W, float* con, void* stream) {
  if (h == nullptr || inputs == nullptr || uv == nullptr || con == nullptr) return fail(BSR_ERR_ARG, "bsr_forward_rgb: null argument");
  if (!h->var.rgb)
    return fail(BSR_ERR_ARG, h->var.tsm ? "bsr_forward_rgb: this handle holds TSM weights: call bsr_forward_tsm"
                                        : "bsr_forward_rgb: this handle holds GSC weights: call bsr_forward");
  if (B <= 0) return fail(BSR_ERR_ARG, "bsr_forward_rgb: B must be positive");
  int rc = BSR_CHECK_IMAGE_SIZE("bsr_forward_rgb", H, W);
  if (rc != BSR_OK) return rc;
  hipStream_t s = static_cast<hipStream_t>(stream);
  DeviceGuard guard(h->device);
  HIP_TRY(guard.err);
  rc = ensure_workspace(h, B, H, W, s);
  if (rc != BSR_OK) return rc;
  h->ev_used = 0;
  h->att_in_lds = false;
  const Plan& p = h->plan;
  float* ws = h->ws;
  const size_t npix = (size_t)B * H * W, ncell = npix / 64;
  const int H2 = H / 2, W2 = W / 2, H4 = H / 4, W4 = W / 4, H8 = H / 8, W8 = W / 8;
  Launcher L{h, s};
  auto glue_begin = [&](const char* what) { L.begin(K_GLUE, what); };
  auto glue_end = [&](const char* what) { L.check(hipGetLastError(), what); L.end(); };

  L.stem(inputs, H, W, ws + p.x1);
  L.conv<3, 3, 2, false, 2, 16, 1>(K_CONV3, "down1", ws + p.x1, 32, 0, 32, H, W, ws + p.c3, RGB_CS_C3, 128, 64, 1);
  L.conv<3, 3, 2, false, 2, 16, 1>(K_CONV3, "down2", ws + p.c3, RGB_CS_C3, 128, 64, H2, W2, ws + p.c2, RGB_CS_C2, 192, 64, 1);
  L.conv<3, 3, 2, false, 3, 16, 1>(K_CONV3, "down3", ws + p.c2, RGB_CS_C2, 192, 64, H4, W4, ws + p.xa, RGB_CS_A, 0, 96, 1);
  glue_begin("uv_resize8");
  hipLaunchKernelGGL(bsr::uv_resize8_kernel, dim3((unsigned)((ncell * 3 + 255) / 256)), dim3(256), 0, s, uv, H, W, ws + p.xa, RGB_CS_A, 96,
                     ws + p.xa, RGB_CS_A, 96, ncell);
  glue_end("uv_resize8");

  auto res_block = [&](int i, const float* x, int x_cs) {
    char nm[32];
    float* y3 = ws + p.y3[i];
    snprintf(nm, sizeof nm, "res%d.conv1", i);
    L.conv<1, 1, 1, false, 2, 32, 3>(K_CONV1, nm, x, x_cs, 0, x_cs, H8, W8, ws + p.t1, RGB_D, 0, RGB_D, 1);
    snprintf(nm, sizeof nm, "res%d.conv2", i);
    L.conv<3, 3, 1, false, 2, 32, 1>(K_CONV3, nm, ws + p.t1, RGB_D, 0, RGB_D, H8, W8, ws + p.t2, RGB_D, 0, RGB_D, 1);
    snprintf(nm, sizeof nm, "res%d.c3q", i);
    L.gemm<3, 8, 1>(K_CONV1, nm, ws + p.t2, RGB_D, ncell, y3, RGB_CS_R, RGB_CS_R + 3 * RGB_D, 0, x, x_cs, x_cs, ws + p.qkv, 3 * RGB_D, RGB_CS_R,
                    RGB_CS_R);
    if (L.rc == BSR_OK) {
      snprintf(nm, sizeof nm, "res%d.attention", i);
      L.begin(K_ATT, nm);
      L.check(bsr::launch_nonlocal_attention256(ws + p.qkv, ws + p.att[i], B, H8 * W8, s), "attention256");
      L.end();
    }
    snprintf(nm, sizeof nm, "res%d.w", i);
    L.gemm<3, 8, 1>(K_CONV1, nm, ws + p.att[i], RGB_D, ncell, ws + p.r[i], RGB_CS_R, RGB_CS_R, 1, y3, RGB_CS_R, RGB_CS_R);
  };
  res_block(0, ws + p.xa, RGB_CS_A);
  res_block(1, ws + p.r[0], RGB_CS_R);
  res_block(2, ws + p.r[1], RGB_CS_R);

  L.conv<3, 3, 1, true, 2, 32, 1>(K_CONVT, "up1", ws + p.r[2], RGB_CS_R, 0, RGB_CS_R, H8, W8, ws + p.c2, RGB_CS_C2, 0, 192, 1);
  L.conv<3, 3, 1, true, 2, 32, 1>(K_CONVT_NI2, "up2", ws + p.c2, RGB_CS_C2, 0, RGB_CS_C2, H4, W4, ws + p.c3, RGB_CS_C3, 0, 128, 1);
  L.conv<3, 3, 1, true, 2, 32, 1>(K_CONVT_NI2, "up3", ws + p.c3, RGB_CS_C3, 0, RGB_CS_C3, H2, W2, ws + p.ybuf, 128, 0, 128, 1);
  L.conv71("rgb_head", ws + p.ybuf, 128, 128, H, W, ws + p.qh, RGB_CS_QH);
  if (L.rc == BSR_OK) {
    glue_begin("rgb_hsum");
    hipLaunchKernelGGL(bsr::rgb_hsum_kernel, dim3((unsigned)((npix * 3 + 255) / 256)), dim3(256), 0, s, ws + p.qh, RGB_CS_QH, h->rgb_head_b, W,
                       ws + p.yh, npix);
    glue_end("rgb_hsum");
    L.begin(K_CONV7, "rgb_tail");
    L.check(bsr::launch_rgb_conv7(ws + p.yh, h->rgb_tail_w, B, H, W, con, ws + p.con, s), "rgb_tail");
    L.end();
  }
  if (L.rc == BSR_OK) h->ran = true;
  return L.rc;
}

int bsr_forward(bsr_handle* h, const float* inputs, const float* uv, int B, int H, int W, float* gs, float* con_rgb, float* mask22,
                float* dif, void* stream) {
  return forward_impl(h, inputs, uv, nullptr, 1, 0, B, H, W, gs, con_rgb, mask22, dif, stream);
}

int bsr_forward_packed(bsr_handle* h, const float* inputs, const float* uv, int B, int H, int W, float* gs, float* con_rgb_dif, float* mask22,
                       void* stream) {
  if (con_rgb_dif == nullptr) return fail(BSR_ERR_ARG, "bsr_forward_packed: null con_rgb_dif");
  return forward_impl(h, inputs, uv, nullptr, 1, 0, B, H, W, gs, nullptr, mask22, nullptr, stream, con_rgb_dif);
}

int bsr_forward_tsm(bsr_handle* h, const float* inputs, const float* uv, const float* reg, int B, int H, int W, int frame, int share,
                    float* gs, float* con_rgb, float* mask22, float* dif, void* stream) {
  if (reg == nullptr) return fail(BSR_ERR_ARG, "bsr_forward_tsm: null reg");
  return forward_impl(h, inputs, uv, reg, frame, share != 0, B, H, W, gs, con_rgb, mask22, dif, stream);
}

int bsr_prep_rows(int device, const void* d_blob, size_t blob_bytes, size_t rows_off, size_t grid_off, int B, int S, float* out, float* hull_tmp,
                  void* stream) {
  if (d_blob == nullptr || out == nullptr || hull_tmp == nullptr) return fail(BSR_ERR_ARG, "bsr_prep_rows: null argument");
  if (B <= 0 || S <= 0 || (S * S) % 256 != 0) return fail(BSR_ERR_ARG, "bsr_prep_rows: B must be positive and S*S a multiple of 256");
  if (rows_off % 8 != 0 || grid_off % 8 != 0) return fail(BSR_ERR_ARG, "bsr_prep_rows: table offsets must be 8-byte aligned");
  if (rows_off > blob_bytes || (size_t)B * sizeof(bsr::PrepRow) > blob_bytes - rows_off || grid_off > blob_bytes ||
      (size_t)S * sizeof(double) > blob_bytes - grid_off)
    return fail(BSR_ERR_ARG, "bsr_prep_rows: the row / grid tables do not fit in blob_bytes");
  DeviceGuard guard(device);
  HIP_TRY(guard.err);
  hipStream_t s = static_cast<hipStream_t>(stream);
  const unsigned char* blob = static_cast<const unsigned char*>(d_blob);
  const dim3 grid((unsigned)(S * S / 256), (unsigned)B);
  hipLaunchKernelGGL(bsr::prep_rows_kernel, grid, dim3(256), 0, s, blob, reinterpret_cast<const bsr::PrepRow*>(blob + rows_off),
                     reinterpret_cast<const double*>(blob + grid_off), S, out, hull_tmp);
  HIP_TRY(hipGetLastError());
  hipLaunchKernelGGL(bsr::prep_blur_kernel, grid, dim3(256), 0, s, hull_tmp, S, 16, out);
  HIP_TRY(hipGetLastError());
  return BSR_OK;
}

int bsr_prep_groups(int device, const void* d_blob, size_t blob_bytes, size_t groups_off, size_t grid_off, int B, int S, int planes, float* out,
                    float* hull_tmp, void* stream) {
  if (d_blob == nullptr || out == nullptr || hull_tmp == nullptr) return fail(BSR_ERR_ARG, "bsr_prep_groups: null argument");
  if (B <= 0 || S <= 0 || (S * S) % 256 != 0) return fail(BSR_ERR_ARG, "bsr_prep_groups: B must be positive and S*S a multiple of 256");
  if (planes != 6 && planes != 7) return fail(BSR_ERR_ARG, "bsr_prep_groups: planes must be 6 (img3, gt3) or 7 (img3, cmap3, label1)");
  if (groups_off % 8 != 0 || grid_off % 8 != 0) return fail(BSR_ERR_ARG, "bsr_prep_groups: table offsets must be 8-byte aligned");
  if (groups_off > blob_bytes || (size_t)B * sizeof(bsr::PrepGroup) > blob_bytes - groups_off || grid_off > blob_bytes ||
      (size_t)S * sizeof(double) > blob_bytes - grid_off)
    return fail(BSR_ERR_ARG, "bsr_prep_groups: the group / grid tables do not fit in blob_bytes");
  DeviceGuard guard(device);
  HIP_TRY(guard.err);
  hipStream_t s = static_cast<hipStream_t>(stream);
  const unsigned char* blob = static_cast<const unsigned char*>(d_blob);
  const bsr::PrepGroup* groups = reinterpret_cast<const bsr::PrepGroup*>(blob + groups_off);
  const double* lin = reinterpret_cast<const double*>(blob + grid_off);
  const dim3 grid((unsigned)(S * S / 256), (unsigned)B);
  if (planes == 6)
    hipLaunchKernelGGL(bsr::prep_groups_kernel<6>, grid, dim3(256), 0, s, blob, groups, lin, S, out, hull_tmp);
  else
    hipLaunchKernelGGL(bsr::prep_groups_kernel<7>, grid, dim3(256), 0, s, blob, groups, lin, S, out, hull_tmp);
  HIP_TRY(hipGetLastError());
  hipLaunchKernelGGL(bsr::prep_blur_kernel, dim3((unsigned)(S * S / 256), 2u * (unsigned)B), dim3(256), 0, s, hull_tmp, S, planes + 10, out);
  HIP_TRY(hipGetLastError());
  return BSR_OK;
}

int bsr_png_unfilter(int device, void* d_blob, size_t blob_bytes, size_t items_off, int n, void* stream) {
  if (d_blob == nullptr) return fail(BSR_ERR_ARG, "bsr_png_unfilter: null argument");
  if (n <= 0 || items_off % 8 != 0) return fail(BSR_ERR_ARG, "bsr_png_unfilter: n must be positive and items_off 8-byte aligned");
  if (items_off > blob_bytes || (size_t)n * sizeof(bsr::UnfilterItem) > blob_bytes - items_off)
    return fail(BSR_ERR_ARG, "bsr_png_unfilter: the item table does not fit in blob_bytes");
  DeviceGuard guard(device);
  HIP_TRY(guard.err);
  unsigned char* blob = static_cast<unsigned char*>(d_blob);
  hipLaunchKernelGGL(bsr::png_unfilter_kernel, dim3((unsigned)n), dim3(256), 0, static_cast<hipStream_t>(stream), blob,
                     reinterpret_cast<const bsr::UnfilterItem*>(blob + items_off));
  HIP_TRY(hipGetLastError());
  return BSR_OK;
}

int bsr_png_unfilter_tall(int device, void* d_blob, size_t blob_bytes, size_t items_off, int n, void* stream) {
  if (d_blob == nullptr) return fail(BSR_ERR_ARG, "bsr_png_unfilter_tall: null argument");
  if (n <= 0 || n > 65535 || items_off % 8 != 0) return fail(BSR_ERR_ARG, "bsr_png_unfilter_tall: n must be 1..65535 and items_off 8-byte aligned");
  if (items_off > blob_bytes || (size_t)n * sizeof(bsr::UnfilterTallItem) > blob_bytes - items_off)
    return fail(BSR_ERR_ARG, "bsr_png_unfilter_tall: the item table does not fit in blob_bytes");
  DeviceGuard guard(device);
  HIP_TRY(guard.err);
  unsigned char* blob = static_cast<unsigned char*>(d_blob);
  hipStream_t s = static_cast<hipStream_t>(stream);
  std::vector<bsr::UnfilterTallItem> items;
  if (int rc = read_records(blob, items_off, n, s, &items)) return rc;
  const long long total = (long long)blob_bytes, slack = bsr::kUnfilterSlack;
  for (int i = 0; i < n; ++i) {
    const bsr::UnfilterTallItem& it = items[(size_t)i];
    const bool shape = (it.c == 1 || it.c == 3 || it.c == 4) && it.h >= 1 && it.h <= 65535 && it.w >= 1 && it.w <= 65535 && (long long)it.w * it.c >= 4 &&
                       it.rows_needed >= 0 && (it.grey_out == 0 || it.c == 1);
    if (!shape) return fail(BSR_ERR_ARG, "bsr_png_unfilter_tall: a record needs c in {1,3,4}, 1 <= h, w <= 65535, w c >= 4, rows_needed >= 0, grey_out with c = 1 only");
    const long long raw = (long long)it.h * (1 + (long long)it.w * it.c), outb = (long long)it.h * it.w * (it.grey_out ? 1 : 3);
    if (it.raw_off < slack || it.raw_off > total || raw + slack > total - it.raw_off || it.out_off < 0 || it.out_off > total || outb + slack > total - it.out_off)
      return fail(BSR_ERR_ARG, "bsr_png_unfilter_tall: a record points outside the blob (16 bytes of the blob must surround the scanlines and follow the output)");
  }
  hipLaunchKernelGGL(bsr::png_unfilter_tall_kernel, dim3((unsigned)n), dim3(256), 0, s, blob, reinterpret_cast<const bsr::UnfilterTallItem*>(blob + items_off));
  HIP_TRY(hipGetLastError());
  return BSR_OK;
}

int bsr_crop_faces(int device, void* d_blob, size_t blob_bytes, size_t items_off, int n, int S, void* stream) {
  if (d_blob == nullptr) return fail(BSR_ERR_ARG, "bsr_crop_faces: null argument");
  if (n <= 0 || n > 65535 || items_off % 8 != 0) return fail(BSR_ERR_ARG, "bsr_crop_faces: n must be 1..65535 and items_off 8-byte aligned");
  if (S != 32 && S != 64 && S != 128 && S != 256) return fail(BSR_ERR_ARG, "bsr_crop_faces: S must be 32, 64, 128 or 256");
  if (items_off > blob_bytes || (size_t)n * sizeof(bsr::CropItem) > blob_bytes - items_off)
    return fail(BSR_ERR_ARG, "bsr_crop_faces: the item table does not fit in blob_bytes");
  DeviceGuard guard(device);
  HIP_TRY(guard.err);
  unsigned char* blob = static_cast<unsigned char*>(d_blob);
  hipStream_t s = static_cast<hipStream_t>(stream);
  std::vector<bsr::CropItem> items;
  if (int rc = read_records(blob, items_off, n, s, &items)) return rc;
  const long long total = (long long)blob_bytes, outb = 3ll * S * S;
  for (int i = 0; i < n; ++i) {
    const bsr::CropItem& it = items[(size_t)i];
    if (it.h < 1 || it.h > 65535 || it.w < 1 || it.w > 65535 || it.preset_x < 0 || it.preset_y < 0 || it.preset_x > (1 << 20) || it.preset_y > (1 << 20))
      return fail(BSR_ERR_ARG, "bsr_crop_faces: a record needs 1 <= h, w <= 65535 and presets in 0..2^20");
    const long long srcb = 3ll * it.h * it.w;
    if (it.src_off < 0 || it.src_off > total || srcb > total - it.src_off || it.out_off < 0 || it.out_off > total || outb > total - it.out_off)
      return fail(BSR_ERR_ARG, "bsr_crop_faces: a record points outside the blob");
    const bool padded = it.preset_x != 0 || it.preset_y != 0;
    const long long cw = padded ? (long long)it.w + 2ll * it.preset_x + 2 : it.w, ch = padded ? (long long)it.h + 2ll * it.preset_y + 2 : it.h;
    if (it.box[0] < 0 || it.box[1] < 0 || it.box[2] <= it.box[0] || it.box[3] <= it.box[1] || it.box[2] > cw || it.box[3] > ch)
      return fail(BSR_ERR_ARG, "bsr_crop_faces: a record's box is empty or leaves its canvas");
  }
  hipLaunchKernelGGL(bsr::crop_faces_kernel, dim3((unsigned)((S / 16) * (S / 16)), (unsigned)n), dim3(256), 0, s, blob,
                     reinterpret_cast<const bsr::CropItem*>(blob + items_off), S);
  HIP_TRY(hipGetLastError());
  return BSR_OK;
}

size_t bsr_png_file_bytes(int H, int W) {
  bsr::PngGeom g;
  return bsr::png_geometry(H, W, &g) ? (size_t)g.file_bytes : 0;
}

size_t bsr_png_scratch_bytes(int B) { return B > 0 ? (size_t)B * bsr::kPngSub * 4 * sizeof(unsigned long long) : 0; }

int bsr_png_encode(int device, const unsigned char* pixels, int B, int H, int W, unsigned char* out, size_t out_stride, void* scratch, void* stream) {
  if (pixels == nullptr || out == nullptr || scratch == nullptr) return fail(BSR_ERR_ARG, "bsr_png_encode: null argument");
  bsr::PngGeom g;
  if (B <= 0 || !bsr::png_geometry(H, W, &g)) return fail(BSR_ERR_ARG, "bsr_png_encode: B, H, W must be positive, W <= 5461 and H <= 65535");
  if (out_stride < g.file_bytes) return fail(BSR_ERR_ARG, "bsr_png_encode: out_stride is smaller than bsr_png_file_bytes(H, W)");
  if (reinterpret_cast<uintptr_t>(scratch) % 8 != 0) return fail(BSR_ERR_ARG, "bsr_png_encode: scratch must be 8-byte aligned");
  DeviceGuard guard(device);
  HIP_TRY(guard.err);
  bsr::PngFigs none{};
  HIP_TRY(bsr::launch_png_encode(pixels, none, B, g, out, out_stride, static_cast<unsigned long long*>(scratch), static_cast<hipStream_t>(stream)));
  return BSR_OK;
}

int bsr_png_encode_figs(int device, int n_figs, const float* const* figs, const float* const* muls, const float* scales, const int* channels,
                        const int* pixel_strides, const int* mul_strides, int B, int H, int Wf, unsigned char* out, size_t out_stride, void* scratch,
                        void* stream) {
  if (figs == nullptr || channels == nullptr || pixel_strides == nullptr || out == nullptr || scratch == nullptr)
    return fail(BSR_ERR_ARG, "bsr_png_encode_figs: null argument");
  if (n_figs < 1 || n_figs > bsr::kPngMaxFigs) return fail(BSR_ERR_ARG, "bsr_png_encode_figs: 1 to 8 figures per strip");
  bsr::PngGeom g;
  if (B <= 0 || Wf <= 0 || !bsr::png_geometry(H, n_figs * Wf, &g))
    return fail(BSR_ERR_ARG, "bsr_png_encode_figs: B, H, Wf must be positive, the strip's width n_figs * Wf <= 5461 and H <= 65535");
  if (out_stride < g.file_bytes) return fail(BSR_ERR_ARG, "bsr_png_encode_figs: out_stride is smaller than bsr_png_file_bytes(H, n_figs * Wf)");
  if (reinterpret_cast<uintptr_t>(scratch) % 8 != 0) return fail(BSR_ERR_ARG, "bsr_png_encode_figs: scratch must be 8-byte aligned");
  bsr::PngFigs f{};
  f.n = n_figs;
  f.Wf = Wf;
  for (int k = 0; k < n_figs; ++k) {
    if (figs[k] == nullptr || (channels[k] != 1 && channels[k] != 3) || pixel_strides[k] < channels[k])
      return fail(BSR_ERR_ARG, "bsr_png_encode_figs: every figure needs a pointer, 1 or 3 channels and a pixel stride of at least its channels");
    f.ptr[k] = figs[k];
    f.mul[k] = muls != nullptr ? muls[k] : nullptr;
    f.scale[k] = scales != nullptr ? scales[k] : 1.f;
    f.ch[k] = channels[k];
    f.ps[k] = pixel_strides[k];
    f.mps[k] = (mul_strides != nullptr && f.mul[k] != nullptr) ? mul_strides[k] : 1;
    if (f.mul[k] != nullptr && f.mps[k] < 1) return fail(BSR_ERR_ARG, "bsr_png_encode_figs: a multiplier needs a positive pixel stride");
  }
  DeviceGuard guard(device);
  HIP_TRY(guard.err);
  HIP_TRY(bsr::launch_png_encode(nullptr, f, B, g, out, out_stride, static_cast<unsigned long long*>(scratch), static_cast<hipStream_t>(stream)));
  return BSR_OK;
}

size_t bsr_ucb_post_scratch_bytes(int B, int S) { return post_size_ok(B, S) ? (size_t)B * bsr::ucb_item_scratch_bytes(S) : 0; }

int bsr_ucb_post(int device, const float* rows10, const unsigned char* masks, const float* boxes, int B, int S, float* losses,
                 unsigned char* strips, float* figs, int* status, void* scratch, void* stream) {
  return run_post("bsr_ucb_post", {rows10, masks, boxes, losses, strips, status, scratch}, B, S, scratch, device, [&] {
    HIP_TRY(bsr::launch_ucb_post(rows10, masks, boxes, B, S, losses, strips, figs, status, scratch, static_cast<hipStream_t>(stream)));
    return BSR_OK;
  });
}

size_t bsr_ucb_post_rgb_scratch_bytes(int B, int S) { return post_size_ok(B, S) ? (size_t)B * bsr::ucb_rgb_item_scratch_bytes(S) : 0; }

int bsr_ucb_post_rgb(int device, const float* rows9, const unsigned char* masks, const float* boxes, int B, int S, float* losses,
                     unsigned char* strips, float* figs, int* status, void* scratch, void* stream) {
  return run_post("bsr_ucb_post_rgb", {rows9, masks, boxes, losses, strips, status, scratch}, B, S, scratch, device, [&] {
    HIP_TRY(bsr::launch_ucb_post_rgb(rows9, masks, boxes, B, S, losses, strips, figs, status, scratch, static_cast<hipStream_t>(stream)));
    return BSR_OK;
  });
}

size_t bsr_ucb_post_tsm_scratch_bytes(int B, int S) { return post_size_ok(B, S) ? (size_t)B * bsr::ucb_tsm_item_scratch_bytes(S) : 0; }

int bsr_ucb_post_tsm(int device, const float* rows, const unsigned char* masks, const float* boxes, int B, int S, float* losses,
                     double* nose_stats, unsigned char* strips, float* figs, int* status, void* scratch, void* stream) {
  return run_post("bsr_ucb_post_tsm", {rows, masks, boxes, losses, nose_stats, strips, status, scratch}, B, S, scratch, device, [&] {
    HIP_TRY(bsr::launch_ucb_post_tsm(rows, masks, boxes, B, S, losses, nose_stats, strips, figs, status, scratch, static_cast<hipStream_t>(stream)));
    return BSR_OK;
  });
}

size_t bsr_sfw_score_scratch_bytes(int B, int S) { return post_size_ok(B, S) ? (size_t)B * bsr::sfw_item_scratch_bytes(S) : 0; }

int bsr_sfw_score(int device, const float* rows3, int B, int S, float* losses, double* auc, float* pred, float* label, int* status,
                  void* scratch, void* stream) {
  return run_post("bsr_sfw_score", {rows3, losses, auc, pred, label, status, scratch}, B, S, scratch, device, [&] {
    HIP_TRY(bsr::launch_sfw_score(rows3, B, S, losses, auc, pred, label, status, scratch, static_cast<hipStream_t>(stream)));
    return BSR_OK;
  });
}

int bsr_clock_trace(int device, unsigned long long* out, int samples, int spin, const int* stop, int* taken, void* stream) {
  if (out == nullptr || stop == nullptr || taken == nullptr || samples <= 0 || spin < 0) return fail(BSR_ERR_ARG, "bsr_clock_trace: bad argument");
  DeviceGuard guard(device);
  HIP_TRY(guard.err);
  hipLaunchKernelGGL(bsr::clock_trace_kernel, dim3(1), dim3(64), 0, static_cast<hipStream_t>(stream), out, samples, spin, stop, taken);
  HIP_TRY(hipGetLastError());
  return BSR_OK;
}

int bsr_debug_split_qkv(const float* qkv, void* qkv_split, int B, int tokens, void* stream) {
  if (qkv == nullptr || qkv_split == nullptr) return fail(BSR_ERR_ARG, "bsr_debug_split_qkv: null argument");
  if (B <= 0 || tokens <= 0 || tokens % 128 != 0) return fail(BSR_ERR_ARG, "bsr_debug_split_qkv: tokens must be a positive multiple of 128");
  const size_t pairs = (size_t)B * tokens * 192;
  hipLaunchKernelGGL(bsr::a4_split_qkv_kernel, dim3((unsigned)((pairs + 255) / 256)), dim3(256), 0, static_cast<hipStream_t>(stream), qkv,
                     static_cast<char*>(qkv_split), pairs);
  HIP_TRY(hipGetLastError());
  return BSR_OK;
}

int bsr_debug_attention_split(const void* qkv_split, float* y, int B, int tokens, int pv1, void* stream) {
  if (qkv_split == nullptr || y == nullptr) return fail(BSR_ERR_ARG, "bsr_debug_attention_split: null argument");
  if (B <= 0 || tokens <= 0 || tokens % 128 != 0) return fail(BSR_ERR_ARG, "bsr_debug_attention_split: tokens must be a positive multiple of 128");
  HIP_TRY(bsr::launch_nonlocal_attention_h16(static_cast<const float*>(qkv_split), y, B, tokens, static_cast<hipStream_t>(stream), pv1 != 0));
  return BSR_OK;
}

int bsr_debug_attention_dtype(const float* qkv, float* y, int B, int tokens, int dtype, void* stream) {
  if (qkv == nullptr || y == nullptr) return fail(BSR_ERR_ARG, "bsr_debug_attention: null argument");
  if (B <= 0 || tokens <= 0 || tokens % 128 != 0) return fail(BSR_ERR_ARG, "bsr_debug_attention: tokens must be a positive multiple of 128");
  if (dtype == BSR_DTYPE_F32) {
    HIP_TRY(bsr::launch_nonlocal_attention(qkv, y, B, tokens, static_cast<hipStream_t>(stream)));
  } else if (dtype == BSR_DTYPE_F32X3 || dtype == BSR_DTYPE_F16) {
    void* tmp = nullptr;
    HIP_TRY(hipMalloc(&tmp, (size_t)B * tokens * bsr::kA4TokBytes));
    int rc = bsr_debug_split_qkv(qkv, tmp, B, tokens, stream);
    if (rc == BSR_OK) rc = bsr_debug_attention_split(tmp, y, B, tokens, 0, stream);
    hipError_t e = hipStreamSynchronize(static_cast<hipStream_t>(stream));
    hipFree(tmp);
    if (rc != BSR_OK) return rc;
    HIP_TRY(e);
  } else {
    return fail(BSR_ERR_ARG, "bsr_debug_attention: unknown dtype");
  }
  return BSR_OK;
}

int bsr_debug_attention_qw(const float* qkv, float* y, int B, int tokens, int qw, void* stream) {
  if (qkv == nullptr || y == nullptr) return fail(BSR_ERR_ARG, "bsr_debug_attention_qw: null argument");
  if (B <= 0 || tokens <= 0 || tokens % 128 != 0) return fail(BSR_ERR_ARG, "bsr_debug_attention_qw: tokens must be a positive multiple of 128");
  if (qw != 0 && qw != 1 && qw != 2 && qw != 4) return fail(BSR_ERR_ARG, "bsr_debug_attention_qw: qw must be 0 (automatic), 1, 2 or 4 query waves per workgroup");
  HIP_TRY(bsr::launch_nonlocal_attention(qkv, y, B, tokens, static_cast<hipStream_t>(stream), qw));
  return BSR_OK;
}

int bsr_debug_attention_rgb(const float* qkv, float* y, int B, int tokens, void* stream) {
  if (qkv == nullptr || y == nullptr) return fail(BSR_ERR_ARG, "bsr_debug_attention_rgb: null argument");
  if (B <= 0 || tokens <= 0 || tokens % 32 != 0) return fail(BSR_ERR_ARG, "bsr_debug_attention_rgb: tokens must be a positive multiple of 32");
  HIP_TRY(bsr::launch_nonlocal_attention256(qkv, y, B, tokens, static_cast<hipStream_t>(stream)));
  return BSR_OK;
}

int bsr_debug_wino_conv(const float* x, const float* w, const float* bias, float* y, int B, int H, int W, int nw, void* stream) {
  if (x == nullptr || w == nullptr || bias == nullptr || y == nullptr) return fail(BSR_ERR_ARG, "bsr_debug_wino_conv: null argument");
  if (B <= 0 || H <= 0 || W <= 0 || H % 4 != 0 || W % 32 != 0) return fail(BSR_ERR_ARG, "bsr_debug_wino_conv: H must be a positive multiple of 4 and W of 32");
  if ((long long)B * H * W * 128 * 4 >= (1LL << 31)) return fail(BSR_ERR_ARG, "bsr_debug_wino_conv: tensor too large");
  if (nw != 0 && nw != 2 && nw != 4) return fail(BSR_ERR_ARG, "bsr_debug_wino_conv: nw must be 0 (automatic), 2 or 4 waves per workgroup");
  HIP_TRY(bsr::launch_wino_conv2(wino_args(x, y, w, bias, H, W), B, static_cast<hipStream_t>(stream), nw));
  return BSR_OK;
}

int bsr_debug_wino_filter(const float* direct, float* out) {
  if (direct == nullptr || out == nullptr) return fail(BSR_ERR_ARG, "bsr_debug_wino_filter: null argument");
  wino_filter_transform(direct, out);
  return BSR_OK;
}

int bsr_debug_keys_compose(const float* c3q_w, const float* c3q_b, float* out_w, float* out_b) {
  if (c3q_w == nullptr || c3q_b == nullptr || out_w == nullptr || out_b == nullptr) return fail(BSR_ERR_ARG, "bsr_debug_keys_compose: null argument");
  keys_compose(c3q_w, c3q_b, out_w, out_b);
  return BSR_OK;
}

int bsr_debug_attention(const float* qkv, float* y, int B, int tokens, void* stream) {
  return bsr_debug_attention_dtype(qkv, y, B, tokens, BSR_DTYPE_F32, stream);
}

struct ProbeSrc { size_t off; int hh, ww, cs, coff, c; bool half; };

static int probe_index(const std::string& nm, const char* prefix, int n) {
  const size_t len = strlen(prefix);
  if (nm.size() == len + 1 && nm.compare(0, len, prefix) == 0 && nm[len] >= '0' && nm[len] < '0' + n) return nm[len] - '0';
  return -1;
}

static int probe_src_rgb(const bsr_handle* h, const std::string& nm, ProbeSrc* src) {
  const Plan& p = h->plan;
  const int H = h->H, W = h->W;
  int i;
  if (nm == "x1") *src = {p.x1, H, W, 32, 0, 32};
  else if (nm == "x2") *src = {p.c3, H / 2, W / 2, RGB_CS_C3, 128, 64};
  else if (nm == "x3") *src = {p.c2, H / 4, W / 4, RGB_CS_C2, 192, 64};
  else if (nm == "x0") *src = {p.xa, H / 8, W / 8, RGB_CS_A, 0, 99};
  else if ((i = probe_index(nm, "res", 3)) >= 0) *src = {p.r[i], H / 8, W / 8, RGB_CS_R, 0, 513};
  else if ((i = probe_index(nm, "att", 3)) >= 0) *src = {p.att[i], H / 8, W / 8, RGB_D, 0, RGB_D};
  else if ((i = probe_index(nm, "y3x", 3)) >= 0) *src = {p.y3[i], H / 8, W / 8, RGB_CS_R, 0, 513};
  else if (nm == "up1") *src = {p.c2, H / 4, W / 4, RGB_CS_C2, 0, 192};
  else if (nm == "up2") *src = {p.c3, H / 2, W / 2, RGB_CS_C3, 0, 128};
  else if (nm == "up3") *src = {p.ybuf, H, W, 128, 0, 128};
  else if (nm == "y") *src = {p.yh, H, W, 3, 0, 3};
  else if (nm == "con") *src = {p.con, H, W, 3, 0, 3};
  else return fail(BSR_ERR_STATE, "bsr_probe: unknown probe '" + nm + "' for an RGB handle");
  return BSR_OK;
}

static int probe_src_gsc(const bsr_handle* h, const std::string& nm, ProbeSrc* src) {
  const Plan& p = h->plan;
  const Variant& v = h->var;
  const int H = h->H, W = h->W;
  const bool p16 = h->dtype == BSR_DTYPE_F16;
  int i;
  if (nm == "x1") *src = {p.x1, H, W, 32, 0, 32, p16};
  else if (nm == "x2") *src = {p.c3, H / 2, W / 2, 128, 64, 64, p16};
  else if (nm == "x3") *src = {p.c2, H / 4, W / 4, 160, 96, 64, p16};
  else if (nm == "x0") *src = {p.xa, H / 8, W / 8, v.cs_a, 0, v.c_a};
  else if ((i = probe_index(nm, "res", 6)) >= 0) *src = {p.r[i], H / 8, W / 8, i < 3 ? v.cs_r : v.cs_h, 0, i < 3 ? v.c_r : v.c_h};
  else if ((i = probe_index(nm, "att", 6)) >= 0) {
    if (h->att_in_lds)
      return fail(BSR_ERR_STATE, "bsr_probe: att<i> does not exist for the last forward — attention and the `w` GEMM ran as one launch and the "
                                 "attention output never left LDS (create the handle with BSR_FUSE_ATTW=0 in the environment to probe it)");
    *src = {p.att[i], H / 8, W / 8, 128, 0, 128};
  }
  else if ((i = probe_index(nm, "y3x", 6)) >= 0) *src = {p.y3[i], H / 8, W / 8, CS_Y3X, 0, CS_Y3X};
  else if (nm == "up1") *src = {p.c2, H / 4, W / 4, 160, 0, 96, p16};
  else if (nm == "up2") *src = {p.c3, H / 2, W / 2, 128, 0, 64, p16};
  else if (nm == "y") *src = {p.ybuf, H, W, 64, 0, 64, p16};
  else if (nm == "d32") *src = {p.probe, H / 8, W / 8, 2, 0, 1};
  else if (nm == "bmask") *src = {p.probe, H / 8, W / 8, 2, 1, 1};
  else if (nm == "xh") *src = {p.xh, H / 8, W / 8, v.cs_h, 0, v.c_h};
  else if (nm == "f1") *src = {p.f1, H / 4, W / 4, 128, 0, 128, p16};
  else if (nm == "f2") *src = {p.f2, H / 2, W / 2, 96, 0, 96, p16};
  else if (nm == "f") *src = {p.cf, H, W, CS_CF, 0, 64, p16};
  else return fail(BSR_ERR_STATE, "bsr_probe: unknown probe '" + nm + "'");
  return BSR_OK;
}

int bsr_probe(bsr_handle* h, const char* name, float* dst, size_t cap_floats, int shape4[4], void* stream) {
  if (h == nullptr || name == nullptr || dst == nullptr || shape4 == nullptr) return fail(BSR_ERR_ARG, "bsr_probe: null argument");
  if (!h->ran) return fail(BSR_ERR_STATE, "bsr_probe: no forward has run on this handle");
  DeviceGuard guard(h->device);
  HIP_TRY(guard.err);
  ProbeSrc src{};
  const int rc = h->var.rgb ? probe_src_rgb(h, name, &src) : probe_src_gsc(h, name, &src);
  if (rc != BSR_OK) return rc;
  const size_t npix = (size_t)h->B * src.hh * src.ww;
  shape4[0] = h->B; shape4[1] = src.hh; shape4[2] = src.ww; shape4[3] = src.c;
  if (npix * src.c > cap_floats) return fail(BSR_ERR_ARG, "bsr_probe: destination too small");
  hipLaunchKernelGGL(bsr::slice_copy_kernel, dim3((unsigned)((npix * src.c + 255) / 256)), dim3(256), 0, static_cast<hipStream_t>(stream),
                     h->ws + src.off, src.cs, src.coff, src.c, dst, npix, src.half ? 1 : 0);
  HIP_TRY(hipGetLastError());
  return BSR_OK;
}

}
```

blindshadowremoval_amd/pack.py:

```python
from __future__ import annotations

import struct
from typing import Dict, List, Tuple

import numpy as np

from .weights import BN_EPS, N_RES, check_weights, detect_variant

BLOB_MAGIC = 0x57525342
BLOB_VERSION = 1
_ENTRY = struct.Struct("<40sQQ4i")
_HEADER = struct.Struct("<4I")

TRANSPOSED = ("up1", "up2", "up3", "clr_up1", "clr_up2", "clr_up3")

DTYPES = {"f32": 0, "f16": 1, "f32x3": 2}
H16_LAYERS = ("down1", "down2", "down3", "up1", "up2", "up3", "clr_up1", "clr_up2", "clr_up3") + tuple("res%d.conv2" % i for i in range(6))
W3_LAYERS = ("up1", "up2", "up3", "clr_up1", "clr_up2", "clr_up3") + tuple("res%d.conv2" % i for i in range(6))
X3_LAYERS = tuple("res%d.%s" % (i, n) for i in range(6) for n in ("conv1", "c3q", "w")) + ("heads", "clr_conv1", "conv1")


def geometry(variant: str = "gsc", dtype: str = "f32") -> Dict[str, Tuple[int, int, int]]:
    if variant == "rgb":
        return geometry_rgb(dtype)
    tsm = variant == "tsm"
    h16 = dtype != "f32"
    if tsm:
        k_a, k_r, k_h = (320, 320, 896) if h16 else (312, 312, 888)
    else:
        k_a, k_r, k_h = (128, 288, 288) if h16 else (120, 264, 264)
    cu = 32 if h16 else 24
    g: Dict[str, Tuple[int, int, int]] = {
        "conv1": (32, 32, 32) if h16 else (24, 24, 32), "down1": (16, 32, 64), "down2": (16, 64, 64), "down3": (16, 64, 96),
        "up1": (cu, k_r, 96), "up2": (32, 160, 64), "up3": (32, 128, 64), "heads": (32, 64, 16),
        "clr_up1": (cu, k_h, 128), "clr_up2": (32, 128, 96), "clr_up3": (32, 96, 64), "clr_conv1": (32, 64, 16),
    }
    for i in range(N_RES):
        g["res%d.conv1" % i] = (cu, k_a if i == 0 else (k_r if i < N_RES // 2 else k_h), 128)
        g["res%d.conv2" % i] = (32, 128, 128)
        g["res%d.c3q" % i] = (32, 128, 768)
        g["res%d.w" % i] = (32, 128, 384)
    return g


def geometry_rgb(dtype: str = "f32") -> Dict[str, Tuple[int, int, int]]:
    if dtype != "f32":
        raise ValueError("the RGB baseline is provided in f32 only (dtype 'f32x3' / 'f16' are not)")
    g: Dict[str, Tuple[int, int, int]] = {
        "conv1": (24, 24, 32), "down1": (16, 32, 64), "down2": (16, 64, 64), "down3": (16, 64, 96),
        "up1": (32, 544, 192), "up2": (32, 256, 128), "up3": (32, 192, 128), "rgb_head": (32, 128, 32),
    }
    for i in range(N_RES // 2):
        g["res%d.conv1" % i] = (32, 128 if i == 0 else 544, 256)
        g["res%d.conv2" % i] = (32, 256, 256)
        g["res%d.c3q" % i] = (32, 256, 544 + 768 + 64)
        g["res%d.w" % i] = (32, 256, 544 + 96)
    return g


GEOMETRY = geometry("gsc")


def fold_bn(kernel_tkn: np.ndarray, bias: np.ndarray, bn: Dict[str, np.ndarray] | None):
    k = kernel_tkn.astype(np.float64)
    b = bias.astype(np.float64)
    if bn is None:
        return k, b
    s = bn["gamma"].astype(np.float64) / np.sqrt(bn["moving_variance"].astype(np.float64) + BN_EPS)
    return k * s[None, None, :], (b - bn["moving_mean"].astype(np.float64)) * s + bn["beta"].astype(np.float64)


def _bn(w: Dict[str, np.ndarray], stem: str) -> Dict[str, np.ndarray]:
    return {p: w[stem + "/" + p] for p in ("gamma", "beta", "moving_mean", "moving_variance")}


def pack_taps(kernel_tkn: np.ndarray, bias: np.ndarray, cc: int, k_pad: int, n_pad: int):
    taps, k, n = kernel_tkn.shape
    assert k <= k_pad and n <= n_pad and k_pad % cc == 0
    full = np.zeros((taps, k_pad, n_pad), np.float64)
    full[:, :k, :n] = kernel_tkn
    arr = np.zeros((k_pad // cc, taps, n_pad, cc + 4), np.float32)
    arr[..., :cc] = full.reshape(taps, k_pad // cc, cc, n_pad).transpose(1, 0, 3, 2)
    b = np.zeros(n_pad, np.float32)
    b[:n] = bias
    return arr, b


def pack_taps_h16(kernel_tkn: np.ndarray, bias: np.ndarray, cc: int, k_pad: int, n_pad: int, nsplit: int, swizzle: bool = False):
    taps, k, n = kernel_tkn.shape
    assert k <= k_pad and n <= n_pad and k_pad % cc == 0 and cc % 16 == 0 and nsplit in (1, 2)
    full = np.zeros((taps, k_pad, n_pad), np.float64)
    full[:, :k, :n] = kernel_tkn.astype(np.float32)
    rows = full.reshape(taps, k_pad // cc, cc, n_pad).transpose(1, 0, 3, 2)
    hi = rows.astype(np.float16)
    if not np.all(np.isfinite(hi)):
        raise ValueError("a folded weight exceeds the fp16 range (65504): this layer cannot run in the 16-bit modes")
    planes = [hi]
    if nsplit == 2:
        planes.append((rows - hi.astype(np.float64)).astype(np.float16))
    if swizzle:
        assert nsplit == 2 and cc == 32
        lin = np.concatenate(planes, axis=3).reshape(rows.shape[:3] + (8, 8))
        img = np.empty_like(lin)
        for row in range(n_pad):
            sw = (row >> 1) & 7
            for slot in range(8):
                img[:, :, row, slot ^ sw] = lin[:, :, row, slot]
        img = np.ascontiguousarray(img.reshape(rows.shape[:3] + (64,)))
    else:
        planes.append(np.zeros(rows.shape[:3] + (8,), np.float16))
        img = np.ascontiguousarray(np.concatenate(planes, axis=3))
    arr = img.view(np.float32)
    b = np.zeros(n_pad, np.float32)
    b[:n] = bias
    return arr, b


def pack_w3(kernel_tkn: np.ndarray, bias: np.ndarray, k_pad: int):
    taps, k, n = kernel_tkn.shape
    assert taps == 9 and k <= k_pad and k_pad % 32 == 0
    nblk, nchunk = (n + 63) // 64, k_pad // 32
    full = np.zeros((9, k_pad, nblk * 64), np.float64)
    full[:, :k, :n] = kernel_tkn.astype(np.float32)
    hi = full.astype(np.float16)
    if not np.all(np.isfinite(hi)):
        raise ValueError("a folded weight exceeds the fp16 range (65504): this layer cannot run in the 16-bit modes")
    rows = hi.reshape(9, nchunk, 4, 8, nblk, 64).transpose(4, 1, 0, 5, 2, 3)
    img = np.empty_like(rows)
    for row in range(64):
        sw = (row >> 2) & 3
        for u in range(4):
            img[:, :, :, row, u ^ sw] = rows[:, :, :, row, u]
    arr = np.ascontiguousarray(img.reshape(nblk * nchunk, 9, 64, 32)).view(np.float32)
    b = np.zeros(nblk * 64, np.float32)
    b[:n] = bias
    return arr, b


def pack_w4(kernel_tkn: np.ndarray, bias: np.ndarray):
    taps, k, n = kernel_tkn.shape
    assert taps == 1 and k == 128 and n <= 288
    full = np.zeros((128, 288), np.float64)
    full[:, :n] = kernel_tkn[0].astype(np.float32)
    hi = full.astype(np.float16)
    if not np.all(np.isfinite(hi)):
        raise ValueError("a folded weight exceeds the fp16 range (65504): this layer cannot run in the 16-bit modes")
    lo = (full - hi.astype(np.float64)).astype(np.float16)
    korder = np.array([[32 * dt + 16 * p + 4 * h + (j & 3) + 8 * (j >> 2) for j in range(8)]
                       for dt in range(4) for p in range(2) for h in range(2)])
    img = np.zeros((288, 32, 8), np.float16)
    for row in range(288):
        sw = row & 15
        for c in range(16):
            img[row, c ^ sw] = hi[korder[c], row]
            img[row, 16 + (c ^ sw)] = lo[korder[c], row]
    arr = np.ascontiguousarray(img.reshape(9, 1, 32, 256)).view(np.float32)
    b = np.zeros(288, np.float32)
    b[:n] = bias
    return arr, b


WINO_G = np.array([[1.0, 0.0, 0.0], [0.5, 0.5, 0.5], [0.5, -0.5, 0.5], [0.0, 0.0, 1.0]])
WINO_CC = 16


def wino_filter_transform(kernel_tkn: np.ndarray, dtype=np.float32) -> np.ndarray:
    taps, k, n = kernel_tkn.shape
    assert taps == 9
    g = kernel_tkn.astype(np.float64).reshape(3, 3, k, n)
    return np.einsum("xa,abkn,yb->xykn", WINO_G, g, WINO_G).reshape(16, k, n).astype(dtype)


def pack_wino(kernel_tkn: np.ndarray, bias: np.ndarray):
    taps, k, n = kernel_tkn.shape
    assert k % WINO_CC == 0
    u = wino_filter_transform(kernel_tkn.astype(np.float32))
    arr = np.ascontiguousarray(u.reshape(16, k // WINO_CC, WINO_CC, n).transpose(1, 0, 3, 2))
    return arr, bias.astype(np.float32)


KEYS_N = 288 + 256
KEYS_N_PAD = KEYS_N + 64


def compose_keys(wq: np.ndarray, bq: np.ndarray, wk: np.ndarray):
    wq, wk, bq = wq.astype(np.float64), wk.astype(np.float64), bq.astype(np.float64)
    return wq @ wk.T, bq @ wk.T


def compose_keys_c3q(c3q_w: np.ndarray, c3q_b: np.ndarray):
    assert c3q_w.shape == (4, 1, 768, 36) and c3q_b.shape == (768,)
    kn = c3q_w[:, 0, :, :32].transpose(0, 2, 1).reshape(128, 768)
    a, ab = compose_keys(kn[:, 288:416], c3q_b[288:416], kn[:, 416:544])
    out = np.zeros((4, 1, KEYS_N_PAD, 36), np.float32)
    out[:, :, :288] = c3q_w[:, :, :288]
    out[:, 0, 288:416, :32] = a.astype(np.float32).reshape(4, 32, 128).transpose(0, 2, 1)
    out[:, :, 416:544] = c3q_w[:, :, 544:672]
    b = np.zeros(KEYS_N_PAD, np.float32)
    b[:288], b[288:416], b[416:544] = c3q_b[:288], ab.astype(np.float32), c3q_b[544:672]
    return out, b


def layer_matrices(w: Dict[str, np.ndarray]) -> "Dict[str, Tuple[np.ndarray, np.ndarray]]":
    out: Dict[str, Tuple[np.ndarray, np.ndarray]] = {}

    def hwio(stem):
        k = w[stem + "/kernel"]
        return k.reshape(k.shape[0] * k.shape[1], k.shape[2], k.shape[3])

    k = w["conv1/conv/kernel"]
    out["conv1"] = fold_bn(k.reshape(7, 21, 32), w["conv1/conv/bias"], _bn(w, "conv1/bnorm"))
    for nm in ("down1", "down2", "down3"):
        out[nm] = fold_bn(hwio(nm + "/conv"), w[nm + "/conv/bias"], _bn(w, nm + "/bnorm"))
    for nm in TRANSPOSED:
        k = w[nm + "/conv/kernel"]
        out[nm] = fold_bn(k.reshape(9, k.shape[2], k.shape[3]).transpose(0, 2, 1), w[nm + "/conv/bias"], _bn(w, nm + "/bnorm"))
    k2, k3 = w["conv2/conv/kernel"][..., 0], w["conv3/conv/kernel"][..., 0]
    hk = np.stack([k2, k3], axis=-1)
    out["heads"] = (hk.transpose(0, 2, 1, 3).reshape(7, 64, 14).astype(np.float64), np.zeros(14))
    k, b = fold_bn(hwio("clr_conv1/conv"), w["clr_conv1/conv/bias"], _bn(w, "clr_conv1/bnorm"))
    out["clr_conv1"] = (k[:, 1:, :], b)
    for i in range(N_RES):
        st = "res_stack/%d/" % i
        out["res%d.conv1" % i] = fold_bn(hwio(st + "conv1"), w[st + "conv1/bias"], _bn(w, st + "bnorm1"))
        out["res%d.conv2" % i] = fold_bn(hwio(st + "conv2"), w[st + "conv2/bias"], _bn(w, st + "bnorm2"))
        k3, b3 = fold_bn(hwio(st + "conv3"), w[st + "conv3/bias"], _bn(w, st + "bnorm3"))
        qkv = np.concatenate([hwio(st + "non_local/" + n) for n in ("theta", "phi", "g")], axis=2).astype(np.float64)
        qb = np.concatenate([w[st + "non_local/%s/bias" % n] for n in ("theta", "phi", "g")]).astype(np.float64)
        kc = np.zeros((1, 128, 672))
        bc = np.zeros(672)
        kc[0, :, :257] = k3[0]
        bc[:257] = b3
        kc[0, :, 288:] = k3[0] @ qkv[0]
        bc[288:] = b3 @ qkv[0] + qb
        out["res%d.c3q" % i] = (kc, bc)
        out["res%d.w" % i] = fold_bn(hwio(st + "non_local/w"), w[st + "non_local/w/bias"], _bn(w, st + "non_local/bnorm"))
    return out


def layer_matrices_rgb(w: Dict[str, np.ndarray]) -> "Dict[str, Tuple[np.ndarray, np.ndarray]]":
    out: Dict[str, Tuple[np.ndarray, np.ndarray]] = {}

    def hwio(stem):
        k = w[stem + "/kernel"]
        return k.reshape(k.shape[0] * k.shape[1], k.shape[2], k.shape[3])

    k = w["conv1/conv/kernel"]
    out["conv1"] = fold_bn(k.reshape(7, 21, 32), w["conv1/conv/bias"], _bn(w, "conv1/bnorm"))
    for nm in ("down1", "down2", "down3"):
        out[nm] = fold_bn(hwio(nm + "/conv"), w[nm + "/conv/bias"], _bn(w, nm + "/bnorm"))
    for nm in ("up1", "up2", "up3"):
        k = w[nm + "/conv/kernel"]
        out[nm] = fold_bn(k.reshape(9, k.shape[2], k.shape[3]).transpose(0, 2, 1), w[nm + "/conv/bias"], _bn(w, nm + "/bnorm"))
    k2 = w["conv2/conv/kernel"].astype(np.float64)
    out["rgb_head"] = (k2.transpose(0, 2, 1, 3).reshape(7, 128, 21), np.zeros(21))
    for i in range(N_RES // 2):
        st = "res_stack/%d/" % i
        out["res%d.conv1" % i] = fold_bn(hwio(st + "conv1"), w[st + "conv1/bias"], _bn(w, st + "bnorm1"))
        out["res%d.conv2" % i] = fold_bn(hwio(st + "conv2"), w[st + "conv2/bias"], _bn(w, st + "bnorm2"))
        k3, b3 = fold_bn(hwio(st + "conv3"), w[st + "conv3/bias"], _bn(w, st + "bnorm3"))
        qkv = np.concatenate([hwio(st + "non_local/" + n) for n in ("theta", "phi", "g")], axis=2).astype(np.float64)
        qb = np.concatenate([w[st + "non_local/%s/bias" % n] for n in ("theta", "phi", "g")]).astype(np.float64)
        kc = np.zeros((1, 256, 544 + 768))
        bc = np.zeros(544 + 768)
        kc[0, :, :513] = k3[0]
        bc[:513] = b3
        kc[0, :, 544:] = k3[0] @ qkv[0]
        bc[544:] = b3 @ qkv[0] + qb
        out["res%d.c3q" % i] = (kc, bc)
        out["res%d.w" % i] = fold_bn(hwio(st + "non_local/w"), w[st + "non_local/w/bias"], _bn(w, st + "non_local/bnorm"))
    return out


def rgb_tail_weights(w: Dict[str, np.ndarray]) -> np.ndarray:
    return np.concatenate([w["conv3/conv/kernel"].reshape(-1), w["conv3/conv/bias"]]).astype(np.float32)


def clr_gs_weights(w: Dict[str, np.ndarray]) -> np.ndarray:
    k, _ = fold_bn(w["clr_conv1/conv/kernel"].reshape(9, 65, 16), w["clr_conv1/conv/bias"], _bn(w, "clr_conv1/bnorm"))
    out = np.zeros((16, 16), np.float32)
    out[:, :9] = k[:, 0, :].T
    return out


def tail_weights(w: Dict[str, np.ndarray]) -> np.ndarray:
    k2, b2 = fold_bn(w["clr_conv2/conv/kernel"].reshape(1, 16, 16), w["clr_conv2/conv/bias"], _bn(w, "clr_conv2/bnorm"))
    k3 = w["clr_conv3/conv/kernel"].reshape(16, 3).astype(np.float64)
    return np.concatenate([k2.reshape(-1), b2, k3.reshape(-1), w["clr_conv3/conv/bias"].astype(np.float64)]).astype(np.float32)


def pack_generator(weights: Dict[str, np.ndarray], dtype: str = "f32") -> bytes:
    if dtype not in DTYPES:
        raise ValueError("dtype must be one of %s" % sorted(DTYPES))
    variant = detect_variant(weights)
    check_weights(weights, variant)
    if variant == "rgb":
        return _pack_rgb(weights, dtype)
    geo = geometry(variant, dtype)
    entries: List[Tuple[str, np.ndarray, Tuple[int, int, int, int]]] = []
    for name, (k, b) in layer_matrices(weights).items():
        cc, k_pad, n_pad = geo[name]
        if dtype != "f32" and name in H16_LAYERS:
            arr, bias = pack_taps_h16(k, b, cc, k_pad, n_pad, 2 if dtype == "f32x3" else 1, swizzle=(dtype == "f32x3" and cc == 32))
        elif dtype != "f32" and name in X3_LAYERS:
            arr, bias = pack_taps_h16(k, b, cc, k_pad, n_pad, 2)
        else:
            arr, bias = pack_taps(k, b, cc, k_pad, n_pad)
        entries.append((name + ".w", arr, tuple(arr.shape)))
        entries.append((name + ".b", bias, (n_pad, 0, 0, 0)))
        if dtype == "f16" and name in W3_LAYERS:
            arr3, bias3 = pack_w3(k, b, k_pad)
            entries.append((name + ".w3.w", arr3, tuple(arr3.shape)))
            entries.append((name + ".w3.b", bias3, (bias3.shape[0], 0, 0, 0)))
        if dtype != "f32" and name.startswith("res") and name.endswith(".w"):
            arr4, bias4 = pack_w4(k, b)
            entries.append((name + "4.w", arr4, tuple(arr4.shape)))
            entries.append((name + "4.b", bias4, (288, 0, 0, 0)))
    entries.append(("heads.bias", np.array([weights["conv2/conv/bias"][0], weights["conv3/conv/bias"][0]], np.float32), (2, 0, 0, 0)))
    entries.append(("clr_conv1.gs", clr_gs_weights(weights), (16, 16, 0, 0)))
    entries.append(("tail.w", tail_weights(weights), (323, 0, 0, 0)))
    return _write_blob(entries, dtype)


def _pack_rgb(weights: Dict[str, np.ndarray], dtype: str) -> bytes:
    geo = geometry_rgb(dtype)
    entries: List[Tuple[str, np.ndarray, Tuple[int, int, int, int]]] = []
    for name, (k, b) in layer_matrices_rgb(weights).items():
        cc, k_pad, n_pad = geo[name]
        arr, bias = pack_taps(k, b, cc, k_pad, n_pad)
        entries.append((name + ".w", arr, tuple(arr.shape)))
        entries.append((name + ".b", bias, (n_pad, 0, 0, 0)))
    entries.append(("rgb.head_bias", weights["conv2/conv/bias"].astype(np.float32), (3, 0, 0, 0)))
    entries.append(("rgb.tail", rgb_tail_weights(weights), (444, 0, 0, 0)))
    return _write_blob(entries, dtype)


def _write_blob(entries, dtype: str) -> bytes:
    off = _HEADER.size + _ENTRY.size * len(entries)
    off = (off + 255) & ~255
    table = bytearray()
    chunks = []
    for name, arr, dims in entries:
        raw = np.ascontiguousarray(arr, dtype="<f4").tobytes()
        table += _ENTRY.pack(name.encode(), off, arr.size, *dims)
        chunks.append((off, raw))
        off = (off + len(raw) + 255) & ~255
    blob = bytearray(off)
    blob[:_HEADER.size] = _HEADER.pack(BLOB_MAGIC, BLOB_VERSION, len(entries), DTYPES[dtype])
    blob[_HEADER.size:_HEADER.size + len(table)] = table
    for o, raw in chunks:
        blob[o:o + len(raw)] = raw
    return bytes(blob)
```

include/bsr_hip.h:

```cpp
#ifndef BSR_HIP_H_
#define BSR_HIP_H_

#include <stddef.h>

#ifdef __cplusplus
extern "C" {
#endif

typedef struct bsr_handle bsr_handle;

#define BSR_OK 0
#define BSR_ERR_ARG 1
#define BSR_ERR_BLOB 2
#define BSR_ERR_HIP 3
#define BSR_ERR_STATE 4
#define BSR_ERR_RANGE 5

#define BSR_DTYPE_F32 0
#define BSR_DTYPE_F16 1
#define BSR_DTYPE_F32X3 2

int bsr_create(bsr_handle** out, int device, const void* packed_weights, size_t nbytes, int dtype);

int bsr_forward(bsr_handle* h, const float* inputs, const float* uv, int B, int H, int W,
                float* gs, float* con_rgb, float* mask22, float* dif, void* stream);

int bsr_forward_packed(bsr_handle* h, const float* inputs, const float* uv, int B, int H, int W,
                       float* gs, float* con_rgb_dif, float* mask22, void* stream);

int bsr_forward_tsm(bsr_handle* h, const float* inputs, const float* uv, const float* reg, int B, int H, int W, int frame, int share,
                    float* gs, float* con_rgb, float* mask22, float* dif, void* stream);

int bsr_forward_rgb(bsr_handle* h, const float* inputs, const float* uv, int B, int H, int W, float* con, void* stream);

int bsr_check_range(bsr_handle* h, void* stream);
int bsr_peek_range(bsr_handle* h);

size_t bsr_workspace_bytes(int B, int H, int W);
size_t bsr_handle_workspace_bytes(const bsr_handle* h, int B, int H, int W);
int bsr_reserve(bsr_handle* h, int B, int H, int W);

int bsr_probe(bsr_handle* h, const char* name, float* dst, size_t cap_floats, int shape4[4], void* stream);

#define BSR_NUM_CLASSES 7
int bsr_set_timing(bsr_handle* h, int enable);
int bsr_get_timing(bsr_handle* h, float ms_per_class[BSR_NUM_CLASSES], int launches_per_class[BSR_NUM_CLASSES]);
int bsr_timing_launches(bsr_handle* h);
int bsr_timing_entry(bsr_handle* h, int i, char* name, size_t name_cap, float* ms, int* cls);

int bsr_prep_rows(int device, const void* d_blob, size_t blob_bytes, size_t rows_off, size_t grid_off, int B, int S, float* out, float* hull_tmp,
                  void* stream);

int bsr_prep_groups(int device, const void* d_blob, size_t blob_bytes, size_t groups_off, size_t grid_off, int B, int S, int planes, float* out,
                    float* hull_tmp, void* stream);

int bsr_png_unfilter(int device, void* d_blob, size_t blob_bytes, size_t items_off, int n, void* stream);

int bsr_png_unfilter_tall(int device, void* d_blob, size_t blob_bytes, size_t items_off, int n, void* stream);

int bsr_crop_faces(int device, void* d_blob, size_t blob_bytes, size_t items_off, int n, int S, void* stream);

size_t bsr_png_file_bytes(int H, int W);
size_t bsr_png_scratch_bytes(int B);
int bsr_png_encode(int device, const unsigned char* pixels, int B, int H, int W, unsigned char* out, size_t out_stride, void* scratch,
                   void* stream);

int bsr_png_encode_figs(int device, int n_figs, const float* const* figs, const float* const* muls, const float* scales, const int* channels,
                        const int* pixel_strides, const int* mul_strides, int B, int H, int Wf, unsigned char* out, size_t out_stride, void* scratch,
                        void* stream);

size_t bsr_ucb_post_scratch_bytes(int B, int S);
int bsr_ucb_post(int device, const float* rows10, const unsigned char* masks, const float* boxes, int B, int S, float* losses,
                 unsigned char* strips, float* figs, int* status, void* scratch, void* stream);

size_t bsr_ucb_post_rgb_scratch_bytes(int B, int S);
int bsr_ucb_post_rgb(int device, const float* rows9, const unsigned char* masks, const float* boxes, int B, int S, float* losses,
                     unsigned char* strips, float* figs, int* status, void* scratch, void* stream);

size_t bsr_sfw_score_scratch_bytes(int B, int S);
int bsr_sfw_score(int device, const float* rows3, int B, int S, float* losses, double* auc, float* pred, float* label, int* status,
                  void* scratch, void* stream);

size_t bsr_ucb_post_tsm_scratch_bytes(int B, int S);
int bsr_ucb_post_tsm(int device, const float* rows, const unsigned char* masks, const float* boxes, int B, int S, float* losses,
                     double* nose_stats, unsigned char* strips, float* figs, int* status, void* scratch, void* stream);

int bsr_debug_attention(const float* qkv, float* y, int B, int tokens, void* stream);
int bsr_debug_attention_rgb(const float* qkv, float* y, int B, int tokens, void* stream);
int bsr_debug_attention_dtype(const float* qkv, float* y, int B, int tokens, int dtype, void* stream);
int bsr_debug_split_qkv(const float* qkv, void* qkv_split, int B, int tokens, void* stream);
int bsr_debug_attention_split(const void* qkv_split, float* y, int B, int tokens, int pv1, void* stream);
int bsr_debug_attention_qw(const float* qkv, float* y, int B, int tokens, int qw, void* stream);
int bsr_debug_wino_conv(const float* x, const float* w, const float* bias, float* y, int B, int H, int W, int nw, void* stream);
int bsr_debug_wino_filter(const float* direct, float* out);
int bsr_debug_keys_compose(const float* c3q_w, const float* c3q_b, float* out_w, float* out_b);

int bsr_clock_trace(int device, unsigned long long* out, int samples, int spin, const int* stop, int* taken, void* stream);

void bsr_destroy(bsr_handle* h);

const char* bsr_last_error(void);

int bsr_abi_version(void);

const char* bsr_source_sha(void);

#ifdef __cplusplus
}
#endif
#endif
```

Measured before the change: 6889 images/sec.

## Fold value projection into attention output weights so keys double as values

```diff
diff --git a/blindshadowremoval_amd/_lib.py b/blindshadowremoval_amd/_lib.py
--- a/blindshadowremoval_amd/_lib.py
+++ b/blindshadowremoval_amd/_lib.py
@@ -17,6 +17,7 @@
            "bsr_get_timing", "bsr_timing_launches", "bsr_timing_entry", "bsr_handle_workspace_bytes", "bsr_debug_attention", "bsr_debug_attention_dtype", "bsr_debug_attention_qw", "bsr_debug_split_qkv", "bsr_clock_trace", "bsr_debug_attention_split", "bsr_destroy", "bsr_last_error", "bsr_abi_version", "bsr_check_range", "bsr_prep_rows", "bsr_prep_groups", "bsr_png_unfilter", "bsr_forward_packed", "bsr_source_sha", "bsr_peek_range", "bsr_png_file_bytes", "bsr_png_scratch_bytes", "bsr_png_encode", "bsr_png_encode_figs", "bsr_ucb_post_scratch_bytes", "bsr_ucb_post",
            "bsr_forward_rgb", "bsr_debug_attention_rgb", "bsr_ucb_post_rgb_scratch_bytes", "bsr_ucb_post_rgb",
            "bsr_sfw_score_scratch_bytes", "bsr_sfw_score", "bsr_ucb_post_tsm_scratch_bytes", "bsr_ucb_post_tsm", "bsr_debug_wino_conv", "bsr_debug_wino_filter", "bsr_debug_keys_compose",
+           "bsr_debug_values_compose",
            "bsr_png_unfilter_tall", "bsr_crop_faces")
 
 
@@ -138,6 +139,10 @@
         raise RuntimeError("libbsr_hip.so has no bsr_debug_keys_compose: rebuild (`python -c 'import __graft_entry__ as g; g.build()'`); "
                            "there is no fallback") from None
     lib.bsr_debug_keys_compose.restype = c_i
+    lib.bsr_debug_values_compose.argtypes = [c_v, c_v, c_v, c_v, c_v, c_v]
+    lib.bsr_debug_values_compose.restype = c_i
+    lib.bsr_debug_attention_kv1.argtypes = [c_v, c_v, c_i, c_i, c_i, c_v]
+    lib.bsr_debug_attention_kv1.restype = c_i
     lib.bsr_peek_range.argtypes = [c_v]
     lib.bsr_peek_range.restype = c_i
     lib.bsr_destroy.argtypes = [c_v]
diff --git a/blindshadowremoval_amd/csrc/attention.h b/blindshadowremoval_amd/csrc/attention.h
--- a/blindshadowremoval_amd/csrc/attention.h
+++ b/blindshadowremoval_amd/csrc/attention.h
@@ -25,9 +25,13 @@
 static_assert(kAttWSmemBytes <= 160 * 1024 && kAttWSmemBytes >= kAttSmemBytes, "LDS budget of the fused tail");
 static_assert(4 * 66 * 64 <= kTailAFloats && kTailLdA == kAttLdK, "the merge scratch sits under the attention tile, clear of the weight ring");
 
-template <int QW, bool FUSEW = false>
+template <int QW, bool FUSEW = false, bool KV1 = false>
 __global__ __launch_bounds__(QW * 128, QW == 4 ? 2 : 1) void nonlocal_attention_kernel(const float* __restrict__ qkv, float* __restrict__ out, int tokens, AttWArgs wa) {
   static_assert(!FUSEW || QW == 4, "the fused w tail is the 8-wave shape's");
+  constexpr int RS = (KV1 ? 2 : 3) * kAttD;
+  constexpr int STAGE = KV1 ? kAttKT * kAttLdK : kAttStageFloats;
+  constexpr int LDV = KV1 ? kAttLdK : kAttD;
+  static_assert(QW * 66 * 64 <= 4 * STAGE, "merge scratch fits the staging buffers");
   extern __shared__ __attribute__((aligned(16))) float smem[];
   constexpr int NT = QW * 128;
   constexpr int SV = 2048 / NT;
@@ -49,7 +53,7 @@
       qb = b % qblocks;
     }
   }
-  const float* base = qkv + (size_t)img * tokens * (3 * kAttD);
+  const float* base = qkv + (size_t)img * tokens * RS;
   const int q = qb * (QW * 32) + wq * 32 + r;
 #if BSR_ATT_PRIO
   if (grp == (BSR_ATT_PRIO - 1)) __builtin_amdgcn_s_setprio(2); else __builtin_amdgcn_s_setprio(0);
@@ -58,7 +62,7 @@
   f32x4 qf[kAttD / 8];
 #pragma unroll
   for (int g = 0; g < kAttD / 8; ++g)
-    qf[g] = *reinterpret_cast<const f32x4*>(base + (size_t)q * (3 * kAttD) + g * 8 + 4 * h) * 1.4426950408889634f;
+    qf[g] = *reinterpret_cast<const f32x4*>(base + (size_t)q * RS + g * 8 + 4 * h) * 1.4426950408889634f;
 
   f32x16 o[4];
 #pragma unroll
@@ -69,21 +73,21 @@
 
   constexpr int V4_PER_TILE = kAttKT * kAttD / 4;
   constexpr int NV = V4_PER_TILE / NT;
-  f32x4 kreg[SV], vreg[SV];
+  f32x4 kreg[SV], vreg[KV1 ? 1 : SV];
   typedef unsigned u32x4_t __attribute__((ext_vector_type(4)));
   const __amdgpu_buffer_rsrc_t kv_rsrc = make_rsrc(base);
   unsigned kv_voff[NV];
 #pragma unroll
   for (int i = 0; i < NV; ++i) {
     const int idx = (tid + i * NT) & (V4_PER_TILE - 1);
-    kv_voff[i] = (unsigned)(((idx / (kAttD / 4)) * (3 * kAttD) + (idx % (kAttD / 4)) * 4) * 4);
+    kv_voff[i] = (unsigned)(((idx / (kAttD / 4)) * RS + (idx % (kAttD / 4)) * 4) * 4);
   }
   auto fetch = [&](int pr) {
 #pragma unroll
     for (int i = 0; i < SV; ++i) {
-      const unsigned soff = (unsigned)((2 * pr + (i / NV)) * kAttKT * (3 * kAttD) * 4);
+      const unsigned soff = (unsigned)((2 * pr + (i / NV)) * kAttKT * RS * 4);
       kreg[i] = __builtin_bit_cast(f32x4, (u32x4_t)__builtin_amdgcn_raw_buffer_load_b128(kv_rsrc, kv_voff[i % NV] + (unsigned)(kAttD * 4), soff, 0));
-      vreg[i] = __builtin_bit_cast(f32x4, (u32x4_t)__builtin_amdgcn_raw_buffer_load_b128(kv_rsrc, kv_voff[i % NV] + (unsigned)(2 * kAttD * 4), soff, 0));
+      if constexpr (!KV1) vreg[i] = __builtin_bit_cast(f32x4, (u32x4_t)__builtin_amdgcn_raw_buffer_load_b128(kv_rsrc, kv_voff[i % NV] + (unsigned)(2 * kAttD * 4), soff, 0));
     }
   };
   auto publish = [&](int pbuf) {
@@ -91,10 +95,9 @@
     for (int i = 0; i < SV; ++i) {
       const int idx = (tid + i * NT) & (V4_PER_TILE - 1), sel = (tid + i * NT) >> 10;
       const int key = idx / (kAttD / 4), c4 = idx % (kAttD / 4);
-      float* sk = smem + (2 * pbuf + sel) * kAttStageFloats;
-      float* sv = sk + kAttKT * kAttLdK;
+      float* sk = smem + (2 * pbuf + sel) * STAGE;
       *reinterpret_cast<f32x4*>(sk + key * kAttLdK + c4 * 4) = kreg[i];
-      *reinterpret_cast<f32x4*>(sv + key * kAttD + c4 * 4) = vreg[i];
+      if constexpr (!KV1) *reinterpret_cast<f32x4*>(sk + kAttKT * kAttLdK + key * kAttD + c4 * 4) = vreg[i];
     }
   };
 
@@ -106,8 +109,8 @@
   auto pair_step = [&](int pr, auto pbuf_const) {
     constexpr int pbuf = decltype(pbuf_const)::value;
     if (pr + 1 < npair) fetch(pr + 1);
-    const float* sk = smem + (2 * pbuf + grp) * kAttStageFloats;
-    const float* sv = sk + kAttKT * kAttLdK;
+    const float* sk = smem + (2 * pbuf + grp) * STAGE;
+    const float* sv = KV1 ? sk : sk + kAttKT * kAttLdK;
 
     f32x16 s;
 #pragma unroll
@@ -147,7 +150,7 @@
 #pragma unroll
     for (int i = 0; i < 16; ++i) {
       const int key = (i & 3) + 8 * (i >> 2) + 4 * h;
-      const f32x4 vf = *reinterpret_cast<const f32x4*>(sv + key * kAttD + 4 * r);
+      const f32x4 vf = *reinterpret_cast<const f32x4*>(sv + key * LDV + 4 * r);
 #pragma unroll
       for (int dt = 0; dt < 4; ++dt) o[dt] = __builtin_amdgcn_mfma_f32_32x32x2f32(vf[dt], s[i], o[dt], 0, 0, 0);
     }
@@ -219,9 +222,9 @@
   }
 }
 
-template <int QW>
+template <int QW, bool KV1 = false>
 inline hipError_t launch_nonlocal_attention_qw(const float* qkv, float* out, int batch, int tokens, hipStream_t stream) {
-  auto kern = nonlocal_attention_kernel<QW, false>;
+  auto kern = nonlocal_attention_kernel<QW, false, KV1>;
   static PerDeviceOnce once;
   const int dev = PerDeviceOnce::current();
   if (dev < 0 || !once.done[dev]) {
@@ -246,9 +249,10 @@
   return qw;
 }
 
+template <bool KV1 = false>
 inline hipError_t launch_nonlocal_attention_w(const float* qkv, int batch, int tokens, const AttWArgs& wa, hipStream_t stream) {
   if (tokens % (4 * kAttKT) != 0 || wa.n_pad * 32 < AttWCfg::BIAS_FLOATS * 32 || wa.n_pad < 12 * 32 || wa.n_store > 288 || wa.res_c > 288 || wa.out2 != nullptr) return hipErrorInvalidValue;
-  auto kern = nonlocal_attention_kernel<4, true>;
+  auto kern = nonlocal_attention_kernel<4, true, KV1>;
   static PerDeviceOnce once;
   const int dev = PerDeviceOnce::current();
   if (dev < 0 || !once.done[dev]) {
@@ -260,12 +264,13 @@
   return hipGetLastError();
 }
 
+template <bool KV1 = false>
 inline hipError_t launch_nonlocal_attention(const float* qkv, float* out, int batch, int tokens, hipStream_t stream, int qw = 0) {
   if (tokens % (4 * kAttKT) != 0) return hipErrorInvalidValue;
   if (qw == 0) qw = attention_auto_qw(batch, tokens);
-  if (qw == 4) return launch_nonlocal_attention_qw<4>(qkv, out, batch, tokens, stream);
-  if (qw == 2) return launch_nonlocal_attention_qw<2>(qkv, out, batch, tokens, stream);
-  if (qw == 1) return launch_nonlocal_attention_qw<1>(qkv, out, batch, tokens, stream);
+  if (qw == 4) return launch_nonlocal_attention_qw<4, KV1>(qkv, out, batch, tokens, stream);
+  if (qw == 2) return launch_nonlocal_attention_qw<2, KV1>(qkv, out, batch, tokens, stream);
+  if (qw == 1) return launch_nonlocal_attention_qw<1, KV1>(qkv, out, batch, tokens, stream);
   return hipErrorInvalidValue;
 }
 
diff --git a/blindshadowremoval_amd/csrc/bsr_api.hip b/blindshadowremoval_amd/csrc/bsr_api.hip
--- a/blindshadowremoval_amd/csrc/bsr_api.hip
+++ b/blindshadowremoval_amd/csrc/bsr_api.hip
@@ -166,6 +166,9 @@
   float* d_blob = nullptr;
   float* d_wino = nullptr;
   float* d_keys = nullptr;
+  float* d_values = nullptr;
+  float* att_scratch = nullptr;
+  size_t att_scratch_floats = 0;
   std::unordered_map<std::string, LayerW> layers;
   Variant var = kGSC;
   int dtype = BSR_DTYPE_F32;
@@ -188,6 +191,8 @@
   bool fuse_attw = true;
   bool wino_conv2 = true;
   bool keys_conv2 = true;
+  bool values_conv2 = true;
+  bool att_is_o = false;
   bool timing = false;
   std::vector<hipEvent_t> ev;
   std::vector<int> ev_class;
@@ -244,6 +249,40 @@
     for (int c = 0; c < 128; ++c) acc += (double)c3q_b[288 + c] * (double)src(m, 416 + c);
     out_b[288 + m] = (float)acc;
   }
+}
+
+constexpr int kWNPad = 384;
+constexpr int kValuesN = 288 + 128, kValuesNPad = kValuesN + 64;
+constexpr int kGProbeNPad = 128 + 64;
+constexpr size_t kValuesWFloats = (size_t)4 * kWNPad * 36 + kWNPad, kValuesC3qFloats = (size_t)4 * kValuesNPad * 36 + kValuesNPad,
+                 kGProbeFloats = (size_t)4 * kGProbeNPad * 36 + kGProbeNPad;
+constexpr size_t kValuesFloats = kValuesWFloats + kValuesC3qFloats + kGProbeFloats;
+void values_compose(const float* c3q_w, const float* c3q_b, const float* w_w, const float* w_b, float* out_w, float* out_b) {
+  auto wg = [&](int k, int c) -> double { return (double)c3q_w[((size_t)(k / 32) * kC3qNPad + 544 + c) * 36 + k % 32]; };
+  auto ww = [&](int c, int n) -> double { return (double)w_w[((size_t)(c / 32) * kWNPad + n) * 36 + c % 32]; };
+  memset(out_w, 0, (size_t)4 * kWNPad * 36 * sizeof(float));
+  for (int n = 0; n < kWNPad; ++n) {
+    for (int k = 0; k < 128; ++k) {
+      double acc = 0.0;
+      for (int c = 0; c < 128; ++c) acc += wg(k, c) * ww(c, n);
+      out_w[((size_t)(k / 32) * kWNPad + n) * 36 + k % 32] = (float)acc;
+    }
+    double acc = (double)w_b[n];
+    for (int c = 0; c < 128; ++c) acc += (double)c3q_b[544 + c] * ww(c, n);
+    out_b[n] = (float)acc;
+  }
+}
+void values_cut(const float* keys_w, const float* keys_b, const float* c3q_w, const float* c3q_b, float* v_w, float* v_b, float* g_w, float* g_b) {
+  memset(v_w, 0, (size_t)4 * kValuesNPad * 36 * sizeof(float));
+  memset(v_b, 0, kValuesNPad * sizeof(float));
+  memset(g_w, 0, (size_t)4 * kGProbeNPad * 36 * sizeof(float));
+  memset(g_b, 0, kGProbeNPad * sizeof(float));
+  for (int ch = 0; ch < 4; ++ch) {
+    memcpy(v_w + (size_t)ch * kValuesNPad * 36, keys_w + (size_t)ch * kKeysNPad * 36, (size_t)kValuesN * 36 * sizeof(float));
+    memcpy(g_w + (size_t)ch * kGProbeNPad * 36, c3q_w + ((size_t)ch * kC3qNPad + 544) * 36, (size_t)128 * 36 * sizeof(float));
+  }
+  memcpy(v_b, keys_b, kValuesN * sizeof(float));
+  memcpy(g_b, c3q_b + 544, 128 * sizeof(float));
 }
 
 int find_layer(bsr_handle* h, const char* name, int nchunk, int taps, int ldp, int n_min, LayerW* out) {
@@ -600,7 +639,7 @@
   h->att_pv1 = dtype == BSR_DTYPE_F16;
   const struct { const char* env; bool* on; } switches[] = {{"BSR_FUSE_HEADS", &h->fuse_heads}, {"BSR_FUSE_ATTW", &h->fuse_attw}, {"BSR_CONV3_F16", &h->conv3_f16},
                                                             {"BSR_CONV1_GEMM", &h->conv1_gemm}, {"BSR_WINO_CONV2", &h->wino_conv2},
-                                                            {"BSR_KEYS_CONV2", &h->keys_conv2}};
+                                                            {"BSR_KEYS_CONV2", &h->keys_conv2}, {"BSR_VALUES_CONV2", &h->values_conv2}};
   for (const auto& sw : switches)
     if (const char* e_ = getenv(sw.env)) *sw.on = atoi(e_) != 0;
   hipError_t e = hipMalloc(reinterpret_cast<void**>(&h->d_blob), nbytes);
@@ -694,6 +733,24 @@
     e = hipMalloc(reinterpret_cast<void**>(&h->d_keys), q.size() * sizeof(float));
     if (e == hipSuccess) e = hipMemcpy(h->d_keys, q.data(), q.size() * sizeof(float), hipMemcpyHostToDevice);
     if (e != hipSuccess) { bsr_destroy(h); return fail(BSR_ERR_HIP, std::string("bsr_create: composed c3q weights: ") + hipGetErrorString(e)); }
+    std::vector<float> v(6 * kValuesFloats);
+    for (int i = 0; i < 6; ++i) {
+      char nm[32];
+      LayerW l, lw;
+      snprintf(nm, sizeof nm, "res%d.c3q", i);
+      if (find_layer(h, nm, 4, 1, 36, kC3qNPad, &l) != BSR_OK) { bsr_destroy(h); return BSR_ERR_BLOB; }
+      snprintf(nm, sizeof nm, "res%d.w", i);
+      if (find_layer(h, nm, 4, 1, 36, kWNPad, &lw) != BSR_OK || lw.n_pad != kWNPad) { bsr_destroy(h); return fail(BSR_ERR_BLOB, std::string("bsr_create: layer '") + nm + "' is not a [4][1][384][36] image"); }
+      float* vw = v.data() + i * kValuesFloats;
+      float* vc = vw + kValuesWFloats;
+      float* vg = vc + kValuesC3qFloats;
+      const float* kq = q.data() + i * kKeysFloats;
+      values_compose(host(l.w), host(l.b), host(lw.w), host(lw.b), vw, vw + (size_t)4 * kWNPad * 36);
+      values_cut(kq, kq + (size_t)4 * kKeysNPad * 36, host(l.w), host(l.b), vc, vc + (size_t)4 * kValuesNPad * 36, vg, vg + (size_t)4 * kGProbeNPad * 36);
+    }
+    e = hipMalloc(reinterpret_cast<void**>(&h->d_values), v.size() * sizeof(float));
+    if (e == hipSuccess) e = hipMemcpy(h->d_values, v.data(), v.size() * sizeof(float), hipMemcpyHostToDevice);
+    if (e != hipSuccess) { bsr_destroy(h); return fail(BSR_ERR_HIP, std::string("bsr_create: composed w weights: ") + hipGetErrorString(e)); }
   }
   *out = h;
   return BSR_OK;
@@ -707,6 +764,8 @@
   if (h->d_blob) hipFree(h->d_blob);
   if (h->d_wino) hipFree(h->d_wino);
   if (h->d_keys) hipFree(h->d_keys);
+  if (h->d_values) hipFree(h->d_values);
+  if (h->att_scratch) hipFree(h->att_scratch);
   if (h->range_flag) hipHostFree(h->range_flag);
   delete h;
 }
@@ -855,14 +914,22 @@
     snprintf(nm, sizeof nm, "res%d.conv1", i);
     if (!conv1_gemm(nm, x, x_cs)) L.conv<1, 1, 1, false, 2, 24, 3>(K_CONV1, nm, x, x_cs, 0, x_cs, H8, W8, ws + p.t1, 128, 0, 128, 1);
     const bool keys = h->dtype == BSR_DTYPE_F32 && h->keys_conv2;
+    const bool values = keys && h->values_conv2;
+    h->att_is_o = values;
     float* t2_row = keys ? ws + p.qkv : ws + p.t2;
-    const int t2_cs = keys ? 384 : 128, t2_coff = keys ? 128 : 0;
+    const int t2_cs = values ? 256 : keys ? 384 : 128, t2_coff = keys ? 128 : 0;
+    const float* vimg = h->d_values + (size_t)i * kValuesFloats;
+    const LayerW lvw{vimg, vimg + (size_t)4 * kWNPad * 36, 4, 1, kWNPad, 36};
     float* t2 = t2_row + t2_coff;
     snprintf(nm, sizeof nm, "res%d.conv2", i);
     if (h->dtype == BSR_DTYPE_F32 && h->wino_conv2) L.wino(nm, i, ws + p.t1, H8, W8, t2, t2_cs);
     else L.conv<3, 3, 1, false, 2, 32, 1>(K_CONV3, nm, ws + p.t1, 128, 0, 128, H8, W8, t2_row, t2_cs, t2_coff, 128, 1);
     snprintf(nm, sizeof nm, "res%d.c3q", i);
-    if (keys) {
+    if (values) {
+      const float* img = vimg + kValuesWFloats;
+      const LayerW lv{img, img + (size_t)4 * kValuesNPad * 36, 4, 1, kValuesNPad, 36};
+      L.gemm<3, 4>(K_CONV1, nm, t2, t2_cs, ncell, y3, CS_Y3X, kValuesN, 0, x, x_cs, x_cs < 288 ? x_cs : 288, ws + p.qkv, 256, 288, CS_Y3X, &lv);
+    } else if (keys) {
       const float* img = h->d_keys + (size_t)i * kKeysFloats;
       const LayerW lk{img, img + (size_t)4 * kKeysNPad * 36, 4, 1, kKeysNPad, 36};
       L.gemm<3, 4>(K_CONV1, nm, t2, t2_cs, ncell, y3, CS_Y3X, kKeysN, 0, x, x_cs, x_cs < 288 ? x_cs : 288, ws + p.qkv, 384, 288, CS_Y3X, &lk, 128, 128);
@@ -876,6 +943,7 @@
       LayerW l;
       snprintf(nm, sizeof nm, h16 ? "res%d.w4" : "res%d.w", i);
       L.rc = h16 ? find_layer(h, nm, 9, 1, 128, 32, &l) : find_layer(h, nm, 4, 1, 36, 12 * 32, &l);
+      if (values) l = lvw;
       if (L.rc == BSR_OK) {
         bsr::AttWArgs wa{};
         wa.w = l.w; wa.bias = l.b; wa.n_pad = h16 ? 288 : l.n_pad;
@@ -883,7 +951,9 @@
         wa.out = r_out; wa.out_cs = o_cs; wa.n_store = o_cs < 288 ? o_cs : 288; wa.n_store1 = wa.n_store; wa.act = 1; wa.stagger = 1;
         snprintf(nm, sizeof nm, "res%d.attw", i);
         L.begin(K_ATT, nm);
-        if (!h16)
+        if (values)
+          L.check(bsr::launch_nonlocal_attention_w<true>(ws + p.qkv, B, H8 * W8, wa, s), "attention+w");
+        else if (!h16)
           L.check(bsr::launch_nonlocal_attention_w(ws + p.qkv, B, H8 * W8, wa, s), "attention+w");
         else
           L.check(bsr::launch_nonlocal_attention_h16_w(ws + p.qkv, B, H8 * W8, wa, s, h->att_pv1), "attention_h16+w");
@@ -893,14 +963,16 @@
       if (L.rc == BSR_OK) {
         snprintf(nm, sizeof nm, "res%d.attention", i);
         L.begin(K_ATT, nm);
-        if (!h16)
+        if (values)
+          L.check(bsr::launch_nonlocal_attention<true>(ws + p.qkv, ws + p.att[i], B, H8 * W8, s), "attention");
+        else if (!h16)
           L.check(bsr::launch_nonlocal_attention(ws + p.qkv, ws + p.att[i], B, H8 * W8, s), "attention");
         else
           L.check(bsr::launch_nonlocal_attention_h16(ws + p.qkv, ws + p.att[i], B, H8 * W8, s, h->att_pv1), "attention_h16");
         L.end();
       }
       snprintf(nm, sizeof nm, "res%d.w", i);
-      L.gemm<3, 4>(K_CONV1, nm, ws + p.att[i], 128, ncell, r_out, o_cs, o_cs < 288 ? o_cs : 288, 1, y3, CS_Y3X, CS_Y3X);
+      L.gemm<3, 4>(K_CONV1, nm, ws + p.att[i], 128, ncell, r_out, o_cs, o_cs < 288 ? o_cs : 288, 1, y3, CS_Y3X, CS_Y3X, nullptr, 0, 0, 0, values ? &lvw : nullptr);
     }
     if (x_c > 288 && L.rc == BSR_OK) {
       glue_begin("lrelu_copy");
@@ -1286,6 +1358,14 @@
   return BSR_OK;
 }
 
+int bsr_debug_attention_kv1(const float* qkv2, float* y, int B, int tokens, int qw, void* stream) {
+  if (qkv2 == nullptr || y == nullptr) return fail(BSR_ERR_ARG, "bsr_debug_attention_kv1: null argument");
+  if (B <= 0 || tokens <= 0 || tokens % 128 != 0) return fail(BSR_ERR_ARG, "bsr_debug_attention_kv1: tokens must be a positive multiple of 128");
+  if (qw != 0 && qw != 1 && qw != 2 && qw != 4) return fail(BSR_ERR_ARG, "bsr_debug_attention_kv1: qw must be 0 (automatic), 1, 2 or 4 query waves per workgroup");
+  HIP_TRY(bsr::launch_nonlocal_attention<true>(qkv2, y, B, tokens, static_cast<hipStream_t>(stream), qw));
+  return BSR_OK;
+}
+
 int bsr_debug_attention_rgb(const float* qkv, float* y, int B, int tokens, void* stream) {
   if (qkv == nullptr || y == nullptr) return fail(BSR_ERR_ARG, "bsr_debug_attention_rgb: null argument");
   if (B <= 0 || tokens <= 0 || tokens % 32 != 0) return fail(BSR_ERR_ARG, "bsr_debug_attention_rgb: tokens must be a positive multiple of 32");
@@ -1314,11 +1394,18 @@
   return BSR_OK;
 }
 
+int bsr_debug_values_compose(const float* c3q_w, const float* c3q_b, const float* w_w, const float* w_b, float* out_w, float* out_b) {
+  if (c3q_w == nullptr || c3q_b == nullptr || w_w == nullptr || w_b == nullptr || out_w == nullptr || out_b == nullptr)
+    return fail(BSR_ERR_ARG, "bsr_debug_values_compose: null argument");
+  values_compose(c3q_w, c3q_b, w_w, w_b, out_w, out_b);
+  return BSR_OK;
+}
+
 int bsr_debug_attention(const float* qkv, float* y, int B, int tokens, void* stream) {
   return bsr_debug_attention_dtype(qkv, y, B, tokens, BSR_DTYPE_F32, stream);
 }
 
-struct ProbeSrc { size_t off; int hh, ww, cs, coff, c; bool half; };
+struct ProbeSrc { size_t off; int hh, ww, cs, coff, c; bool half; int derive; };
 
 static int probe_index(const std::string& nm, const char* prefix, int n) {
   const size_t len = strlen(prefix);
@@ -1361,7 +1448,19 @@
     if (h->att_in_lds)
       return fail(BSR_ERR_STATE, "bsr_probe: att<i> does not exist for the last forward — attention and the `w` GEMM ran as one launch and the "
                                  "attention output never left LDS (create the handle with BSR_FUSE_ATTW=0 in the environment to probe it)");
+    *src = {p.att[i], H / 8, W / 8, 128, 0, 128, false, h->att_is_o ? i + 1 : 0};
+  }
+  else if ((i = probe_index(nm, "attv", 6)) >= 0) {
+    if (!h->att_is_o) return fail(BSR_ERR_STATE, "bsr_probe: attv<i> exists only for a forward with conv2's output as the attention values (fp32, BSR_KEYS_CONV2 and BSR_VALUES_CONV2 on)");
+    if (h->att_in_lds)
+      return fail(BSR_ERR_STATE, "bsr_probe: attv<i> does not exist for the last forward — attention and the `w` GEMM ran as one launch and the "
+                                 "attention output never left LDS (create the handle with BSR_FUSE_ATTW=0 in the environment to probe it)");
     *src = {p.att[i], H / 8, W / 8, 128, 0, 128};
+  }
+  else if (nm == "qkv") {
+    if (h->dtype != BSR_DTYPE_F32) return fail(BSR_ERR_STATE, "bsr_probe: qkv is an fp32 tensor of BSR_DTYPE_F32 handles only");
+    const int c = h->att_is_o ? 256 : 384;
+    *src = {p.qkv, H / 8, W / 8, c, 0, c};
   }
   else if ((i = probe_index(nm, "y3x", 6)) >= 0) *src = {p.y3[i], H / 8, W / 8, CS_Y3X, 0, CS_Y3X};
   else if (nm == "up1") *src = {p.c2, H / 4, W / 4, 160, 0, 96, p16};
@@ -1388,8 +1487,24 @@
   const size_t npix = (size_t)h->B * src.hh * src.ww;
   shape4[0] = h->B; shape4[1] = src.hh; shape4[2] = src.ww; shape4[3] = src.c;
   if (npix * src.c > cap_floats) return fail(BSR_ERR_ARG, "bsr_probe: destination too small");
+  const float* from = h->ws + src.off;
+  if (src.derive) {
+    if (h->att_scratch_floats < npix * 128) {
+      if (h->att_scratch) hipFree(h->att_scratch);
+      h->att_scratch = nullptr;
+      h->att_scratch_floats = 0;
+      HIP_TRY(hipMalloc(reinterpret_cast<void**>(&h->att_scratch), npix * 128 * sizeof(float)));
+      h->att_scratch_floats = npix * 128;
+    }
+    const float* img = h->d_values + (size_t)(src.derive - 1) * kValuesFloats + kValuesWFloats + kValuesC3qFloats;
+    bsr::ConvArgs a{};
+    a.in = from; a.in_cs = 128; a.out = h->att_scratch; a.out_cs = 128;
+    a.w = img; a.bias = img + (size_t)4 * kGProbeNPad * 36; a.nchunk = 4; a.n_pad = kGProbeNPad; a.n_store = 128; a.act = 0;
+    HIP_TRY((bsr::launch_gemm_nloop<3, 4, 0, 2>(a, npix, 2, static_cast<hipStream_t>(stream))));
+    from = h->att_scratch;
+  }
   hipLaunchKernelGGL(bsr::slice_copy_kernel, dim3((unsigned)((npix * src.c + 255) / 256)), dim3(256), 0, static_cast<hipStream_t>(stream),
-                     h->ws + src.off, src.cs, src.coff, src.c, dst, npix, src.half ? 1 : 0);
+                     from, src.cs, src.coff, src.c, dst, npix, src.half ? 1 : 0);
   HIP_TRY(hipGetLastError());
   return BSR_OK;
 }
diff --git a/blindshadowremoval_amd/pack.py b/blindshadowremoval_amd/pack.py
--- a/blindshadowremoval_amd/pack.py
+++ b/blindshadowremoval_amd/pack.py
@@ -199,6 +199,30 @@
     b = np.zeros(KEYS_N_PAD, np.float32)
     b[:288], b[288:416], b[416:544] = c3q_b[:288], ab.astype(np.float32), c3q_b[544:672]
     return out, b
+
+
+VALUES_N = 288 + 128
+VALUES_N_PAD = VALUES_N + 64
+W_N_PAD = 384
+
+
+def compose_values(wg: np.ndarray, bg: np.ndarray, ww: np.ndarray, bw: np.ndarray):
+    wg, bg, ww, bw = (a.astype(np.float64) for a in (wg, bg, ww, bw))
+    w2, b2 = np.zeros((wg.shape[0], ww.shape[1])), bw.copy()
+    for c in range(wg.shape[1]):
+        w2 += wg[:, c:c + 1] * ww[c][None, :]
+        b2 += bg[c] * ww[c]
+    return w2, b2
+
+
+def compose_values_w(c3q_w: np.ndarray, c3q_b: np.ndarray, w_w: np.ndarray, w_b: np.ndarray):
+    assert c3q_w.shape == (4, 1, 768, 36) and c3q_b.shape == (768,) and w_w.shape == (4, 1, W_N_PAD, 36) and w_b.shape == (W_N_PAD,)
+    wg = c3q_w[:, 0, 544:672, :32].transpose(0, 2, 1).reshape(128, 128)
+    ww = w_w[:, 0, :, :32].transpose(0, 2, 1).reshape(128, W_N_PAD)
+    w2, b2 = compose_values(wg, c3q_b[544:672], ww, w_b)
+    out = np.zeros((4, 1, W_N_PAD, 36), np.float32)
+    out[:, 0, :, :32] = w2.astype(np.float32).reshape(4, 32, W_N_PAD).transpose(0, 2, 1)
+    return out, b2.astype(np.float32)
 
 
 def layer_matrices(w: Dict[str, np.ndarray]) -> "Dict[str, Tuple[np.ndarray, np.ndarray]]":
diff --git a/include/bsr_hip.h b/include/bsr_hip.h
--- a/include/bsr_hip.h
+++ b/include/bsr_hip.h
@@ -94,6 +94,8 @@
 int bsr_debug_wino_conv(const float* x, const float* w, const float* bias, float* y, int B, int H, int W, int nw, void* stream);
 int bsr_debug_wino_filter(const float* direct, float* out);
 int bsr_debug_keys_compose(const float* c3q_w, const float* c3q_b, float* out_w, float* out_b);
+int bsr_debug_values_compose(const float* c3q_w, const float* c3q_b, const float* w_w, const float* w_b, float* out_w, float* out_b);
+int bsr_debug_attention_kv1(const float* qkv2, float* y, int B, int tokens, int qw, void* stream);
 
 int bsr_clock_trace(int device, unsigned long long* out, int samples, int spin, const int* stop, int* taken, void* stream);
 
```

Result: faster. 7002 images/sec, median of 6 (+1.6%).
